# klindsay28/NK_ocn_tracer_jacobian_precond

Hardware: AMD Instinct MI355X
Metric: precond_solve_throughput_1deg_ocean_jacobian (higher is better)
Workload: dtype f64

## Files before the change

include/nkp.h:

```cpp
#ifndef NKP_H
#define NKP_H

#include <stdint.h>

#ifdef __cplusplus
extern "C" {
#endif

#define NKP_VERSION 1

typedef struct nkp_solver nkp_solver;

enum nkp_precond {
   NKP_PRECOND_NONE = 0,
   NKP_PRECOND_COLUMN_JACOBI = 1,
   NKP_PRECOND_MULTILEVEL = 3
};

enum nkp_krylov { NKP_KRYLOV_FGMRES = 0, NKP_KRYLOV_BICGSTAB = 1 };

enum {
   NKP_OK = 0,
   NKP_NOT_CONVERGED = 1,
   NKP_BREAKDOWN = 2,
   NKP_OK_BERR = 3,
   NKP_EINVAL = -1,
   NKP_ENOMEM = -2,
   NKP_EDEVICE = -3,
   NKP_ESINGULAR = -4,
   NKP_ECOMM = -5
};

typedef struct nkp_tuning {
   int struct_size;
   int ml_split;
   int ml_pocket;
   int ml_big_from;
   int ml_coarsest_rows;
   int ml_dense_max;
   double ml_theta;
   double ml_tau;
   int64_t ml_device_min;
   int ml_smooth_coarse;
   int ml_coarse_from;
   int ml_gamma_from, ml_gamma_to;
   int ml_f32;
   int ml_host_inverse;
   int ml_fused;
   int ml_fused_max_cols;
   int ml_wave_fused;
   int ml_coarsest_sweeps;
   int64_t ml_tail_rows;
   double ml_omega;
   int col_ldsres;
   int col_stream;
   int col_stream_min;
   int col_stream_gw;
   int col_wave_max;
   int col_w3;
   int col_group;
   int col_pipe_min;
   int col_ldsres_early;
   int col_ldsres_packed;
   int spmv_variant;
   int spmv_compress;
   int spmv_pipe_min;
   int spmv_run;
   int spmv_wgs;
   int rhs_batch;
   int precond_steps;
   int equil;
   int dist_overlap;
   int dist_ras;
   int force_dist;
   int setup_threads;
   int plan_times;
   int ml_drop_intertracer;
   int dist_one_reduce;
   int ml_huge_from;
   int col_ldsres_min;
   int col_sort_groups;
   int batch_spmv_rows;
   int dist_ras_rings;
   int ml_diag;
   int spmv_diag;
   int ml_lane_fused;
   int dist_smooth_exchange;
} nkp_tuning;

int nkp_default_tuning (nkp_tuning *t);

typedef struct nkp_options {
   int struct_size;
   int precond;
   int krylov;
   int restart;
   int max_iters;
   double rtol;
   double atol;
   int device;
   int verbose;
   int rank;
   int reorth;
   int ml_levels;
   int ml_smooth;
   int basis_f32;
   int precond_steps;
   int equil;
   int reserved[4];
   const int32_t *col_i;
   const int32_t *col_j;
   const int32_t *col_t;
   const nkp_tuning *tuning;
} nkp_options;

int nkp_default_options (nkp_options *opt);

int nkp_device_count (void);

int nkp_create (nkp_solver **out, const nkp_options *opt, int64_t n, int64_t nnz,
                const int32_t *rowptr, const int32_t *colind, const double *val,
                const int32_t *blk_start, int64_t nblk, int coupled_tracer_cnt);

int nkp_create64 (nkp_solver **out, const nkp_options *opt, int64_t n, const int64_t *rowptr ,
                  const int32_t *colind, const double *val, const int32_t *blk_start, int64_t nblk, int coupled_tracer_cnt);

int nkp_solve (nkp_solver *s, double *b_in_x_out, int nrhs, int64_t ldb,
               double *berr, int *iters, double *relres);

int nkp_solve_batch_device (nkp_solver *s, int nrhs, const void *d_B, void *d_X, int64_t ldb, double *berr, int *iters, double *relres);

int nkp_solve_device (nkp_solver *s, const void *d_b, void *d_x, int use_guess,
                      double *berr, int *iters, double *relres);

int nkp_spmv (nkp_solver *s, const double *x, double *y);
int nkp_spmv_device (nkp_solver *s, const void *d_x, void *d_y);

int nkp_precond_apply (nkp_solver *s, const double *r, double *z);

int nkp_multi_dot (nkp_solver *s, const double *V, int64_t ld, int k, const double *w, double *out);

int nkp_time_kernel (nkp_solver *s, int which, int arg, int reps, double *avg_ms);

int64_t nkp_get_int (nkp_solver *s, const char *key);

#define NKP_REFACTOR_REBUILD 1
int nkp_refactor (nkp_solver *s, const double *val, int flags);
int nkp_refactor_device (nkp_solver *s, const void *d_val, int flags);

int nkp_refactor_dist (nkp_solver *s, const double *val_loc, int flags);
int nkp_refactor_dist_device (nkp_solver *s, const void *d_val_loc, int flags);

int nkp_set_stream (nkp_solver *s, void *hip_stream);

void nkp_destroy (nkp_solver *s);

const char *nkp_last_error (void);


typedef struct nkp_comm_ops {
   void *ctx;
   int rank, nranks;
   int (*allreduce) (void *ctx, void *dev_buf, int count, int op, void *hip_stream);
   int (*alltoallv) (void *ctx, const void *dev_send, const int *send_counts, void *dev_recv, const int *recv_counts, void *hip_stream);
   int (*alltoallv_i32_host) (void *ctx, const int32_t *send, const int *send_counts, int32_t *recv, const int *recv_counts);
   int (*allgather_i64_host) (void *ctx, int64_t mine, int64_t *all );
} nkp_comm_ops;

int nkp_comm_unique_id (void *id128);
int nkp_comm_rccl_init (nkp_comm_ops *ops, const void *id128, int rank, int nranks);
void nkp_comm_rccl_free (nkp_comm_ops *ops);
int nkp_comm_file_init (nkp_comm_ops *ops, const char *dir, int rank, int nranks);
void nkp_comm_file_free (nkp_comm_ops *ops);

int nkp_create_dist (nkp_solver **out, const nkp_options *opt, int64_t n_global, int64_t fst_row,
                     int64_t m_loc, int64_t nnz_loc, const int32_t *rowptr_loc,
                     const int32_t *colind_glob, const double *val,
                     const int32_t *blk_start_loc, int64_t nblk_loc, int coupled_tracer_cnt,
                     const nkp_comm_ops *comm);

int nkp_cell_major_order (int64_t nblk, const int32_t *blk_start, int cnt, int32_t *perm, int32_t *blk_start_new,
                          int32_t *col_t, int32_t *col_src);
int nkp_permuted_rows (int64_t n, const int32_t *rowptr, const int32_t *colind, const double *val, const int32_t *perm,
                       const int32_t *inv, int64_t r0, int64_t r1, int32_t *rowptr_loc, int32_t *colind_loc, double *val_loc);

int nkp_clone (nkp_solver *src, nkp_solver **out);

int nkp_transpose (nkp_solver *s, nkp_solver **out);

int nkp_transpose_dist (nkp_solver *s, nkp_solver **out);

int nkp_value_gradient_device (nkp_solver *s, int nrhs, const void *d_lambda, const void *d_x, int64_t ld, double alpha, int accumulate, void *d_gval);
int nkp_value_gradient (nkp_solver *s, int nrhs, const double *lambda, const double *x, int64_t ld, double alpha, int accumulate, double *gval);

int nkp_values_product_device (nkp_solver *s, int nrhs, const void *d_val, const void *d_x, int64_t ldx, double alpha, int accumulate, void *d_y, int64_t ldy);
int nkp_values_product (nkp_solver *s, int nrhs, const double *val, const double *x, int64_t ldx, double alpha, int accumulate, double *y, int64_t ldy);

int nkp_solve_tangent_device (nkp_solver *s, int nrhs, const void *d_dval, const void *d_x, int64_t ldx, const void *d_db, void *d_dx, int64_t ld,
                              double *berr, int *iters, double *relres);

int nkp_set_device (int device);

int nkp_gather_root (nkp_solver *s, const double *x_loc, double *x_global);

typedef struct nkp_dist_plan nkp_dist_plan;
int nkp_dist_overlap_plan_host (nkp_dist_plan **out, const nkp_options *opt, int64_t n_global, int64_t fst_row, int64_t m_loc,
                                int64_t nnz_loc, const int32_t *rowptr_loc, const int32_t *colind_glob, const double *val,
                                const int32_t *blk_start_loc, int64_t nblk_loc, int coupled_tracer_cnt, const nkp_comm_ops *comm);
int64_t nkp_dist_plan_size (const nkp_dist_plan *p, const char *what);
int nkp_dist_plan_copy (const nkp_dist_plan *p, const char *what, void *dst);
void nkp_dist_plan_free (nkp_dist_plan *p);

int nkp_dist_plan_host (int64_t m_loc, int64_t nnz_loc, const int32_t *rowptr_loc, const int32_t *colind_glob,
                        int rank, int nranks, const int64_t *starts, int32_t *colind_ext, int32_t *halo_rows,
                        int64_t *n_halo, int32_t *need_counts);

int64_t nkp_ml_level_array (nkp_solver *s, int level, const char *what, void *dst, int64_t capacity_bytes);

int64_t nkp_matrix_array (nkp_solver *s, const char *what, void *dst, int64_t capacity_bytes);

int nkp_ml_plan_host (int64_t n, const int32_t *rowptr, const int32_t *colind, const double *val, const int32_t *blk_start,
                      int64_t nblk, const int32_t *col_i, const int32_t *col_j, int coupled_tracer_cnt, int max_levels,
                      int coarsest_rows, int64_t capacity, int *n_levels, int64_t *rows, int32_t *cmap, int32_t *col_of);

#ifdef __cplusplus
}
#endif
#endif
```

nk_ocn_tracer_jacobian_precond_amd/csrc/blas1.hip:

```cpp
#include "nkp_dev.h"

#include <stdint.h>

#define B1_THREADS 256

__device__ __forceinline__ double wave_sum (double v)
{
#pragma unroll
   for (int off = NKP_WAVE / 2; off > 0; off >>= 1) v += __shfl_down (v, off);
   return v;
}

__device__ __forceinline__ double block_sum (double v, double *sh )
{
   v = wave_sum (v);
   const int lane = threadIdx.x & (NKP_WAVE - 1), wv = threadIdx.x / NKP_WAVE;
   __syncthreads ();
   if (lane == 0) sh[wv] = v;
   __syncthreads ();
   double s = 0.0;
   if (threadIdx.x == 0) {
#pragma unroll
      for (int w = 0; w < B1_THREADS / NKP_WAVE; w++) s += sh[w];
   }
   return s;
}

static inline int red_grid (int64_t n)
{
   int64_t g = (n + 2 * B1_THREADS - 1) / (2 * B1_THREADS);
   if (g < 1) g = 1;
   if (g > NKP_RED_BLOCKS) g = NKP_RED_BLOCKS;
   return (int) g;
}

template <class VT, class VT2>
__device__ __forceinline__ void multi_dot_body (const VT *__restrict__ V, int64_t ld, int k, const double *__restrict__ w,
                                                int64_t n, double *__restrict__ partial, double *sh)
{
   const int chunk = blockIdx.y;
   const int j0 = chunk * NKP_DOT_CHUNK;
   const int kc = (k - j0) < NKP_DOT_CHUNK ? (k - j0) : NKP_DOT_CHUNK;
   const VT *Vc = V + (int64_t) j0 * ld;
   double acc[NKP_DOT_CHUNK];
#pragma unroll
   for (int c = 0; c < NKP_DOT_CHUNK; c++) acc[c] = 0.0;
   double accw = 0.0;
   const int64_t stride = (int64_t) gridDim.x * B1_THREADS * 2;
   for (int64_t i = ((int64_t) blockIdx.x * B1_THREADS + threadIdx.x) * 2; i < n; i += stride) {
      if (i + 1 < n) {
         const double2 w2 = *reinterpret_cast<const double2 *> (w + i);
         accw += w2.x * w2.x + w2.y * w2.y;
#pragma unroll
         for (int c = 0; c < NKP_DOT_CHUNK; c++)
            if (c < kc) {
               const VT2 v2 = *reinterpret_cast<const VT2 *> (Vc + (int64_t) c * ld + i);
               acc[c] += (double) v2.x * w2.x + (double) v2.y * w2.y;
            }
      } else {
         const double w1 = w[i];
         accw += w1 * w1;
#pragma unroll
         for (int c = 0; c < NKP_DOT_CHUNK; c++)
            if (c < kc) acc[c] += (double) Vc[(int64_t) c * ld + i] * w1;
      }
   }
   double *out = partial + ((int64_t) chunk * gridDim.x + blockIdx.x) * (NKP_DOT_CHUNK + 1);
#pragma unroll
   for (int c = 0; c < NKP_DOT_CHUNK; c++) {
      const double s = block_sum (acc[c], sh);
      if (threadIdx.x == 0) out[c] = s;
   }
   const double sw = block_sum (accw, sh);
   if (threadIdx.x == 0) out[NKP_DOT_CHUNK] = sw;
}

template <class VT, class VT2>
__global__ __launch_bounds__ (B1_THREADS)
void multi_dot_kernel (const VT *__restrict__ V, int64_t ld, int k, const double *__restrict__ w,
                       int64_t n, double *__restrict__ partial)
{
   __shared__ double sh[B1_THREADS / NKP_WAVE];
   multi_dot_body<VT, VT2> (V, ld, k, w, n, partial, sh);
}

__global__ __launch_bounds__ (B1_THREADS)
void multi_dot_group_kernel (GsGroup G, int64_t ld, int k, int64_t n)
{
   __shared__ double sh[B1_THREADS / NKP_WAVE];
   const int r = blockIdx.z;
   multi_dot_body<double, double2> (G.V[r], ld, k, G.w[r], n, G.partial[r], sh);
}

__device__ __forceinline__ void multi_dot_finish_body (const double *__restrict__ partial, int nblk, int k, double *__restrict__ out)
{
   const int j = blockIdx.x;
   const int chunk = (j < k) ? j / NKP_DOT_CHUNK : 0;
   const int c = (j < k) ? j % NKP_DOT_CHUNK : NKP_DOT_CHUNK;
   const double *p = partial + (int64_t) chunk * nblk * (NKP_DOT_CHUNK + 1) + c;
   double s = 0.0;
   for (int b = threadIdx.x; b < nblk; b += NKP_WAVE) s += p[(int64_t) b * (NKP_DOT_CHUNK + 1)];
   s = wave_sum (s);
   if (threadIdx.x == 0) out[j] = s;
}

__global__ __launch_bounds__ (NKP_WAVE)
void multi_dot_finish_kernel (const double *__restrict__ partial, int nblk, int k, double *__restrict__ out)
{
   multi_dot_finish_body (partial, nblk, k, out);
}

__global__ __launch_bounds__ (NKP_WAVE)
void multi_dot_finish_group_kernel (GsGroup G, int nblk, int k, double *__restrict__ msg)
{
   multi_dot_finish_body (G.partial[blockIdx.y], nblk, k, msg + (int64_t) blockIdx.y * (k + 1));
}

void launch_multi_dot (const void *V, int v_f32, int64_t ld, int k, const double *w, int64_t n, double *partial, double *out, hipStream_t st)
{
   const int g = red_grid (n);
   const int nchunk = k > 0 ? (k + NKP_DOT_CHUNK - 1) / NKP_DOT_CHUNK : 1;
   if (v_f32) hipLaunchKernelGGL ((multi_dot_kernel<float, float2>), dim3 (g, nchunk), dim3 (B1_THREADS), 0, st, (const float *) V, ld, k, w, n, partial);
   else hipLaunchKernelGGL ((multi_dot_kernel<double, double2>), dim3 (g, nchunk), dim3 (B1_THREADS), 0, st, (const double *) V, ld, k, w, n, partial);
   hipLaunchKernelGGL (multi_dot_finish_kernel, dim3 (k + 1), dim3 (NKP_WAVE), 0, st, partial, g, k, out);
}

void launch_multi_dot_group (int R, const GsGroup &G, int64_t ld, int k, int64_t n, double *msg, hipStream_t st)
{
   if (R <= 0) return;
   const int g = red_grid (n);
   const int nchunk = k > 0 ? (k + NKP_DOT_CHUNK - 1) / NKP_DOT_CHUNK : 1;
   hipLaunchKernelGGL (multi_dot_group_kernel, dim3 (g, nchunk, R), dim3 (B1_THREADS), 0, st, G, ld, k, n);
   hipLaunchKernelGGL (multi_dot_finish_group_kernel, dim3 (k + 1, R), dim3 (NKP_WAVE), 0, st, G, g, k, msg);
}

#define B1_MAX_K NKP_MAX_K
template <class VT, class VT2>
__device__ __forceinline__ void update_w_body (const VT *__restrict__ V, int64_t ld, int k, const double *__restrict__ h,
                                               double *__restrict__ w, int64_t n, double *__restrict__ partial, double sign, double *hs, double *sh)
{
   for (int j = threadIdx.x; j < k; j += B1_THREADS) hs[j] = sign * h[j];
   __syncthreads ();
   double nrm = 0.0;
   const int64_t stride = (int64_t) gridDim.x * B1_THREADS * 2;
   for (int64_t i = ((int64_t) blockIdx.x * B1_THREADS + threadIdx.x) * 2; i < n; i += stride) {
      if (i + 1 < n) {
         double2 a = *reinterpret_cast<const double2 *> (w + i);
         int j = 0;
         for (; j + 4 <= k; j += 4) {
            const VT2 v0 = *reinterpret_cast<const VT2 *> (V + (int64_t) (j + 0) * ld + i);
            const VT2 v1 = *reinterpret_cast<const VT2 *> (V + (int64_t) (j + 1) * ld + i);
            const VT2 v2 = *reinterpret_cast<const VT2 *> (V + (int64_t) (j + 2) * ld + i);
            const VT2 v3 = *reinterpret_cast<const VT2 *> (V + (int64_t) (j + 3) * ld + i);
            a.x += hs[j] * v0.x; a.y += hs[j] * v0.y;
            a.x += hs[j + 1] * v1.x; a.y += hs[j + 1] * v1.y;
            a.x += hs[j + 2] * v2.x; a.y += hs[j + 2] * v2.y;
            a.x += hs[j + 3] * v3.x; a.y += hs[j + 3] * v3.y;
         }
         for (; j < k; j++) {
            const VT2 v0 = *reinterpret_cast<const VT2 *> (V + (int64_t) j * ld + i);
            a.x += hs[j] * v0.x; a.y += hs[j] * v0.y;
         }
         *reinterpret_cast<double2 *> (w + i) = a;
         nrm += a.x * a.x + a.y * a.y;
      } else {
         double a = w[i];
         for (int j = 0; j < k; j++) a += hs[j] * V[(int64_t) j * ld + i];
         w[i] = a;
         nrm += a * a;
      }
   }
   if (partial) {
      const double s = block_sum (nrm, sh);
      if (threadIdx.x == 0) partial[blockIdx.x] = s;
   }
}

template <class VT, class VT2>
__global__ __launch_bounds__ (B1_THREADS)
void update_w_kernel (const VT *__restrict__ V, int64_t ld, int k, const double *__restrict__ h,
                      double *__restrict__ w, int64_t n, double *__restrict__ partial, double sign)
{
   __shared__ double hs[B1_MAX_K];
   __shared__ double sh[B1_THREADS / NKP_WAVE];
   update_w_body<VT, VT2> (V, ld, k, h, w, n, partial, sign, hs, sh);
}

__global__ __launch_bounds__ (B1_THREADS)
void update_w_group_kernel (GsGroup G, int64_t ld, int k, const double *__restrict__ msg, int64_t n)
{
   __shared__ double hs[B1_MAX_K];
   __shared__ double sh[B1_THREADS / NKP_WAVE];
   const int r = blockIdx.y;
   update_w_body<double, double2> (G.V[r], ld, k, msg + (int64_t) r * (k + 1), G.w[r], n, G.partial[r], -1.0, hs, sh);
}

__device__ __forceinline__ void sum_partials_body (const double *__restrict__ partial, int nblk, double *__restrict__ out)
{
   double s = 0.0;
   for (int b = threadIdx.x; b < nblk; b += NKP_WAVE) s += partial[b];
   s = wave_sum (s);
   if (threadIdx.x == 0) out[0] = s;
}

__global__ __launch_bounds__ (NKP_WAVE)
void sum_partials_kernel (const double *__restrict__ partial, int nblk, double *__restrict__ out)
{
   sum_partials_body (partial, nblk, out);
}

__global__ __launch_bounds__ (NKP_WAVE)
void sum_partials_group_kernel (GsGroup G, int nblk, double *__restrict__ out)
{
   sum_partials_body (G.partial[blockIdx.x], nblk, out + blockIdx.x);
}

void launch_update_w (const void *V, int v_f32, int64_t ld, int k, const double *h, double *w, int64_t n, double *partial, double *out_nrm2, hipStream_t st)
{
   const int g = red_grid (n);
   if (v_f32) hipLaunchKernelGGL ((update_w_kernel<float, float2>), dim3 (g), dim3 (B1_THREADS), 0, st, (const float *) V, ld, k, h, w, n, partial, -1.0);
   else hipLaunchKernelGGL ((update_w_kernel<double, double2>), dim3 (g), dim3 (B1_THREADS), 0, st, (const double *) V, ld, k, h, w, n, partial, -1.0);
   hipLaunchKernelGGL (sum_partials_kernel, dim3 (1), dim3 (NKP_WAVE), 0, st, partial, g, out_nrm2);
}

void launch_update_w_group (int R, const GsGroup &G, int64_t ld, int k, const double *msg, int64_t n, double *nrm2, hipStream_t st)
{
   if (R <= 0) return;
   const int g = red_grid (n);
   hipLaunchKernelGGL (update_w_group_kernel, dim3 (g, R), dim3 (B1_THREADS), 0, st, G, ld, k, msg, n);
   hipLaunchKernelGGL (sum_partials_group_kernel, dim3 (R), dim3 (NKP_WAVE), 0, st, G, g, nrm2);
}

void launch_axpy_multi (const double *Z, int64_t ld, int k, const double *c, double *x, int64_t n, hipStream_t st)
{
   const int g = red_grid (n);
   hipLaunchKernelGGL ((update_w_kernel<double, double2>), dim3 (g), dim3 (B1_THREADS), 0, st, Z, ld, k, c, x, n, (double *) nullptr, 1.0);
}

__device__ __forceinline__ void scale_to_body (const double *__restrict__ x, const double *__restrict__ alpha, double *__restrict__ y, float *__restrict__ yf, int64_t n)
{
   const double a = alpha[0];
   const int64_t stride = (int64_t) gridDim.x * B1_THREADS * 2;
   for (int64_t i = ((int64_t) blockIdx.x * B1_THREADS + threadIdx.x) * 2; i < n; i += stride) {
      if (i + 1 < n) {
         double2 v = *reinterpret_cast<const double2 *> (x + i);
         v.x *= a; v.y *= a;
         *reinterpret_cast<double2 *> (y + i) = v;
         if (yf) *reinterpret_cast<float2 *> (yf + i) = make_float2 ((float) v.x, (float) v.y);
      } else {
         y[i] = a * x[i];
         if (yf) yf[i] = (float) (a * x[i]);
      }
   }
}

__global__ __launch_bounds__ (B1_THREADS)
void scale_to_kernel (const double *__restrict__ x, const double *__restrict__ alpha, double *__restrict__ y, float *__restrict__ yf, int64_t n)
{
   scale_to_body (x, alpha, y, yf, n);
}

__global__ __launch_bounds__ (B1_THREADS)
void scale_to_group_kernel (GsGroup G, const double *__restrict__ inv, int64_t n)
{
   const int r = blockIdx.y;
   scale_to_body (G.w[r], inv + r, G.vnext[r], nullptr, n);
}

void launch_scale_to (const double *x, const double *alpha_dev, double *y, float *yf, int64_t n, hipStream_t st)
{
   hipLaunchKernelGGL (scale_to_kernel, dim3 (red_grid (n)), dim3 (B1_THREADS), 0, st, x, alpha_dev, y, yf, n);
}

void launch_scale_to_group (int R, const GsGroup &G, const double *inv, int64_t n, hipStream_t st)
{
   if (R > 0) hipLaunchKernelGGL (scale_to_group_kernel, dim3 (red_grid (n), R), dim3 (B1_THREADS), 0, st, G, inv, n);
}

__global__ __launch_bounds__ (B1_THREADS)
void axpby_kernel (double a, const double *__restrict__ x, double b, double *__restrict__ y, int64_t n)
{
   const int64_t stride = (int64_t) gridDim.x * B1_THREADS;
   for (int64_t i = (int64_t) blockIdx.x * B1_THREADS + threadIdx.x; i < n; i += stride)
      y[i] = (b == 0.0 ? 0.0 : b * y[i]) + (x ? a * x[i] : a);
}

void launch_axpby (double a, const double *x, double b, double *y, int64_t n, hipStream_t st)
{
   hipLaunchKernelGGL (axpby_kernel, dim3 (red_grid (n) * 2), dim3 (B1_THREADS), 0, st, a, x, b, y, n);
}

__global__ __launch_bounds__ (B1_THREADS)
void vmul_kernel (const double *x, const double *__restrict__ w, double *y, int64_t n)
{
   const int64_t stride = (int64_t) gridDim.x * B1_THREADS;
   for (int64_t i = (int64_t) blockIdx.x * B1_THREADS + threadIdx.x; i < n; i += stride) y[i] = x[i] * w[i];
}

void launch_vmul (const double *x, const double *w, double *y, int64_t n, hipStream_t st)
{
   hipLaunchKernelGGL (vmul_kernel, dim3 (red_grid (n) * 2), dim3 (B1_THREADS), 0, st, x, w, y, n);
}

void launch_copy (const double *x, double *y, int64_t n, hipStream_t st)
{
   (void) hipMemcpyAsync (y, x, (size_t) n * sizeof (double), hipMemcpyDeviceToDevice, st);
}

__global__ __launch_bounds__ (B1_THREADS)
void zero_kernel (double *__restrict__ y, int64_t n)
{
   const int64_t stride = (int64_t) gridDim.x * B1_THREADS * 2;
   for (int64_t i = ((int64_t) blockIdx.x * B1_THREADS + threadIdx.x) * 2; i < n; i += stride) {
      if (i + 1 < n) *reinterpret_cast<double2 *> (y + i) = make_double2 (0.0, 0.0);
      else y[i] = 0.0;
   }
}

void launch_fill (double *y, double v, int64_t n, hipStream_t st)
{
   if (n <= 0) return;
   if (v == 0.0) {
      if ((reinterpret_cast<uintptr_t> (y) & 15) == 0) hipLaunchKernelGGL (zero_kernel, dim3 (red_grid (n) * 2), dim3 (B1_THREADS), 0, st, y, n);
      else (void) hipMemsetAsync (y, 0, (size_t) n * sizeof (double), st);
   } else
      launch_axpby (v, nullptr, 0.0, y, n, st);
}

__global__ __launch_bounds__ (B1_THREADS)
void dot_kernel (const double *__restrict__ x, const double *__restrict__ y, int64_t n, double *__restrict__ partial)
{
   __shared__ double sh[B1_THREADS / NKP_WAVE];
   double acc = 0.0;
   const int64_t stride = (int64_t) gridDim.x * B1_THREADS * 2;
   for (int64_t i = ((int64_t) blockIdx.x * B1_THREADS + threadIdx.x) * 2; i < n; i += stride) {
      if (i + 1 < n) {
         const double2 a = *reinterpret_cast<const double2 *> (x + i);
         const double2 b = *reinterpret_cast<const double2 *> (y + i);
         acc += a.x * b.x + a.y * b.y;
      } else
         acc += x[i] * y[i];
   }
   const double s = block_sum (acc, sh);
   if (threadIdx.x == 0) partial[blockIdx.x] = s;
}

void launch_dot (const double *x, const double *y, int64_t n, double *partial, double *out, hipStream_t st)
{
   const int g = red_grid (n);
   hipLaunchKernelGGL (dot_kernel, dim3 (g), dim3 (B1_THREADS), 0, st, x, y, n, partial);
   hipLaunchKernelGGL (sum_partials_kernel, dim3 (1), dim3 (NKP_WAVE), 0, st, partial, g, out);
}

__device__ __forceinline__ double max_or_nan (double q, double m)
{
   return (q > m || q != q) ? q : m;
}

__global__ __launch_bounds__ (B1_THREADS)
void berr_kernel (const double *__restrict__ r, const double *__restrict__ den, int64_t n, double *__restrict__ partial)
{
   __shared__ double sh[B1_THREADS / NKP_WAVE];
   double m = 0.0;
   const int64_t stride = (int64_t) gridDim.x * B1_THREADS;
   for (int64_t i = (int64_t) blockIdx.x * B1_THREADS + threadIdx.x; i < n; i += stride) {
      const double a = fabs (r[i]), d = den[i];
      const double q = (d > 0.0 || d != d) ? a / d : (a != a ? a : a > 0.0 ? 1.0e300 : 0.0);
      m = max_or_nan (q, m);
   }
   for (int off = NKP_WAVE / 2; off > 0; off >>= 1) m = max_or_nan (__shfl_down (m, off), m);
   const int lane = threadIdx.x & (NKP_WAVE - 1), wv = threadIdx.x / NKP_WAVE;
   if (lane == 0) sh[wv] = m;
   __syncthreads ();
   if (threadIdx.x == 0) {
      for (int w = 1; w < B1_THREADS / NKP_WAVE; w++) m = max_or_nan (sh[w], m);
      partial[blockIdx.x] = m;
   }
}

__global__ __launch_bounds__ (NKP_WAVE)
void max_partials_kernel (const double *__restrict__ partial, int nblk, double *__restrict__ out)
{
   double m = 0.0;
   for (int b = threadIdx.x; b < nblk; b += NKP_WAVE) m = max_or_nan (partial[b], m);
   for (int off = NKP_WAVE / 2; off > 0; off >>= 1) m = max_or_nan (__shfl_down (m, off), m);
   if (threadIdx.x == 0) out[0] = m;
}

void launch_berr (const double *r, const double *den, int64_t n, double *partial, double *out, hipStream_t st)
{
   const int g = red_grid (n);
   hipLaunchKernelGGL (berr_kernel, dim3 (g), dim3 (B1_THREADS), 0, st, r, den, n, partial);
   hipLaunchKernelGGL (max_partials_kernel, dim3 (1), dim3 (NKP_WAVE), 0, st, partial, g, out);
}

__global__ __launch_bounds__ (B1_THREADS)
void count_entries_kernel (const double *__restrict__ x, int64_t n, double *__restrict__ partial)
{
   __shared__ double sh[B1_THREADS / NKP_WAVE];
   double bad = 0.0, set = 0.0;
   const int64_t stride = (int64_t) gridDim.x * B1_THREADS;
   for (int64_t i = (int64_t) blockIdx.x * B1_THREADS + threadIdx.x; i < n; i += stride) {
      const double v = x[i];
      bad += (v - v == 0.0) ? 0.0 : 1.0;
      set += (v == 0.0) ? 0.0 : 1.0;
   }
   const double sb = block_sum (bad, sh);
   if (threadIdx.x == 0) partial[blockIdx.x] = sb;
   const double ss = block_sum (set, sh);
   if (threadIdx.x == 0) partial[NKP_RED_BLOCKS + blockIdx.x] = ss;
}

void launch_count_entries (const double *x, int64_t n, double *partial, double *out, hipStream_t st)
{
   const int g = red_grid (n);
   hipLaunchKernelGGL (count_entries_kernel, dim3 (g), dim3 (B1_THREADS), 0, st, x, n, partial);
   hipLaunchKernelGGL (sum_partials_kernel, dim3 (1), dim3 (NKP_WAVE), 0, st, partial, g, out);
   hipLaunchKernelGGL (sum_partials_kernel, dim3 (1), dim3 (NKP_WAVE), 0, st, partial + NKP_RED_BLOCKS, g, out + 1);
}

__device__ __forceinline__ void finish_column_body (double *__restrict__ h, const double *__restrict__ h2, int k,
                                                    const double *__restrict__ nrm2, double *__restrict__ inv)
{
   if (h2)
      for (int j = threadIdx.x; j < k; j += NKP_WAVE) h[j] += h2[j];
   if (threadIdx.x == 0) {
      const double t = sqrt (nrm2[0]);
      h[k] = t;
      inv[0] = (t > 0.0) ? 1.0 / t : 0.0;
   }
}

__global__ __launch_bounds__ (NKP_WAVE)
void finish_column_kernel (double *__restrict__ h, const double *__restrict__ h2, int k,
                           const double *__restrict__ nrm2, double *__restrict__ inv)
{
   finish_column_body (h, h2, k, nrm2, inv);
}

__device__ __forceinline__ void finish_column_pythagoras_body (double *__restrict__ h, int k, double *__restrict__ inv)
{
   double s = 0.0;
   for (int j = threadIdx.x; j < k; j += NKP_WAVE) s += h[j] * h[j];
   for (int off = NKP_WAVE / 2; off > 0; off >>= 1) s += __shfl_down (s, off);
   if (threadIdx.x == 0) {
      const double ww = h[k];
      double t2 = ww - s;
      const bool weak = !(t2 >= 1e-8 * ww);
      if (!(t2 > 0.0)) t2 = 0.0;
      const double t = sqrt (t2);
      h[k] = weak ? -t : t;
      inv[0] = (t > 0.0) ? 1.0 / t : 0.0;
   }
}

__global__ __launch_bounds__ (NKP_WAVE)
void finish_column_pythagoras_kernel (double *__restrict__ h, int k, double *__restrict__ inv)
{
   finish_column_pythagoras_body (h, k, inv);
}

__global__ __launch_bounds__ (NKP_WAVE)
void finish_column_group_kernel (double *__restrict__ msg, const double *__restrict__ msg2, int k, const double *__restrict__ nrm2, double *__restrict__ inv)
{
   const int64_t r = blockIdx.x;
   if (nrm2) finish_column_body (msg + r * (k + 1), msg2 ? msg2 + r * (k + 1) : nullptr, k, nrm2 + r, inv + r);
   else finish_column_pythagoras_body (msg + r * (k + 1), k, inv + r);
}

void launch_finish_column_group (int R, double *msg, const double *msg2, int k, const double *nrm2, double *inv, hipStream_t st)
{
   if (R > 0) hipLaunchKernelGGL (finish_column_group_kernel, dim3 (R), dim3 (NKP_WAVE), 0, st, msg, msg2, k, nrm2, inv);
}

void launch_finish_column_pythagoras (double *h, int k, double *inv, hipStream_t st)
{
   hipLaunchKernelGGL (finish_column_pythagoras_kernel, dim3 (1), dim3 (NKP_WAVE), 0, st, h, k, inv);
}

void launch_finish_column (double *h, const double *h2, int k, const double *nrm2, double *inv, hipStream_t st)
{
   hipLaunchKernelGGL (finish_column_kernel, dim3 (1), dim3 (NKP_WAVE), 0, st, h, h2, k, nrm2, inv);
}

__global__ __launch_bounds__ (B1_THREADS)
void restrict_sum_kernel (const int *__restrict__ rptr, const int *__restrict__ ridx, const double *__restrict__ fine,
                          double *__restrict__ coarse, int64_t nc)
{
   const int64_t stride = (int64_t) gridDim.x * B1_THREADS;
   for (int64_t I = (int64_t) blockIdx.x * B1_THREADS + threadIdx.x; I < nc; I += stride) {
      double acc = 0.0;
      for (int q = rptr[I]; q < rptr[I + 1]; q++) acc += fine[ridx[q]];
      coarse[I] = acc;
   }
}

void launch_restrict_sum (const int *rptr, const int *ridx, const double *fine, double *coarse, int64_t nc, hipStream_t st)
{
   if (nc <= 0) return;
   hipLaunchKernelGGL (restrict_sum_kernel, dim3 (red_grid (nc) * 2), dim3 (B1_THREADS), 0, st, rptr, ridx, fine, coarse, nc);
}

__global__ __launch_bounds__ (B1_THREADS)
void prolong_add_kernel (const int *__restrict__ cmap, const double *__restrict__ coarse, double *__restrict__ fine, int64_t nf, double omega)
{
   const int64_t stride = (int64_t) gridDim.x * B1_THREADS;
   for (int64_t i = (int64_t) blockIdx.x * B1_THREADS + threadIdx.x; i < nf; i += stride) fine[i] += omega * coarse[cmap[i]];
}

void launch_prolong_add (const int *cmap, const double *coarse, double *fine, int64_t nf, double omega, hipStream_t st)
{
   if (nf <= 0) return;
   hipLaunchKernelGGL (prolong_add_kernel, dim3 (red_grid (nf) * 2), dim3 (B1_THREADS), 0, st, cmap, coarse, fine, nf, omega);
}

__global__ __launch_bounds__ (B1_THREADS)
void gather_kernel (const int *__restrict__ perm, const double *__restrict__ in, double *__restrict__ out, int64_t n, int scatter)
{
   const int64_t stride = (int64_t) gridDim.x * B1_THREADS;
   for (int64_t i = (int64_t) blockIdx.x * B1_THREADS + threadIdx.x; i < n; i += stride) {
      if (scatter) out[perm[i]] = in[i];
      else out[i] = in[perm[i]];
   }
}

void launch_gather (const int *perm, const double *in, double *out, int64_t n, hipStream_t st)
{
   if (n <= 0) return;
   hipLaunchKernelGGL (gather_kernel, dim3 (red_grid (n) * 2), dim3 (B1_THREADS), 0, st, perm, in, out, n, 0);
}

void launch_scatter (const int *perm, const double *in, double *out, int64_t n, hipStream_t st)
{
   if (n <= 0) return;
   hipLaunchKernelGGL (gather_kernel, dim3 (red_grid (n) * 2), dim3 (B1_THREADS), 0, st, perm, in, out, n, 1);
}

__global__ __launch_bounds__ (B1_THREADS)
void dense_matvec_kernel (const double *__restrict__ M, const double *__restrict__ x, double *__restrict__ y, int n)
{
   const int row = (int) ((blockIdx.x * B1_THREADS + threadIdx.x) / NKP_WAVE);
   const int lane = threadIdx.x & (NKP_WAVE - 1);
   if (row >= n) return;
   const double *m = M + (int64_t) row * n;
   double acc = 0.0;
   for (int c = lane; c < n; c += NKP_WAVE) acc += m[c] * x[c];
   acc = wave_sum (acc);
   if (lane == 0) y[row] = acc;
}

void launch_dense_matvec (const double *Minv, const double *x, double *y, int n, hipStream_t st)
{
   if (n <= 0) return;
   const int waves_per_block = B1_THREADS / NKP_WAVE;
   hipLaunchKernelGGL (dense_matvec_kernel, dim3 ((n + waves_per_block - 1) / waves_per_block), dim3 (B1_THREADS), 0, st, Minv, x, y, n);
}
```

nk_ocn_tracer_jacobian_precond_amd/csrc/inspect.hip:

```cpp
#include "solver_impl.h"

#include <string.h>

#include <vector>

extern "C" int64_t nkp_ml_level_array (nkp_solver *s, int level, const char *what, void *dst, int64_t capacity_bytes)
{
   if (!s || !what || s->opt.precond != NKP_PRECOND_MULTILEVEL || level < 0 || level >= (int) s->ml.lev.size ()) return fail (NKP_EINVAL, "nkp_ml_level_array: bad argument");
   const MlLevel &V = s->ml.lev[(size_t) level];
   const bool last = level == (int) s->ml.lev.size () - 1;
   const void *src = nullptr;
   int64_t count = 0;
   size_t elem = 4;
   bool host = false;
   int col_kernel[11];
   if (!strcmp (what, "rowptr")) { src = V.L.rowptr; count = V.n + 1; }
   else if (!strcmp (what, "colind")) { src = V.L.colind; count = V.L.nnz; }
   else if (!strcmp (what, "valf")) { src = V.L.valf; count = V.L.valf ? V.L.nnz : 0; }
   else if (!strcmp (what, "val")) { src = V.L.val; count = V.L.val ? V.L.nnz : 0; elem = 8; }
   else if (!strcmp (what, "dg_ptr")) { src = V.L.dg_ptr; count = src ? V.L.dg_ncol + 1 : 0; }
   else if (!strcmp (what, "dg_key")) { src = V.L.dg_key; count = src ? (int64_t) V.L.dg_nkey : 0; }
   else if (!strcmp (what, "dg_voff")) { src = V.L.dg_voff; count = src ? V.L.dg_ncol : 0; elem = 8; }
   else if (!strcmp (what, "dg_val")) { src = V.L.dg_val; count = src ? V.L.dg_nval : 0; }
   else if (!strcmp (what, "dg_gptr")) { src = V.L.dg_gptr; count = src ? V.L.dg_ncol + 1 : 0; }
   else if (!strcmp (what, "dg_grp")) { src = V.L.dg_grp; count = src ? 2 * (int64_t) V.L.dg_ngrp : 0; }
   else if (!strcmp (what, "cmap")) { src = V.cmap; count = V.cmap ? V.n : 0; }
   else if (!strcmp (what, "rptr")) { src = V.rptr; count = V.rptr ? V.nc + 1 : 0; }
   else if (!strcmp (what, "ridx")) { src = V.ridx; count = V.ridx ? V.n : 0; }
   else if (!strcmp (what, "blk_start")) { src = V.B.blk_start; count = V.B.blk_start ? V.B.nblk + 1 : 0; }
   else if (!strcmp (what, "fac")) { src = V.B.fac; count = V.B.fac ? (int64_t) (2 * V.B.P + 1) * V.n : 0; elem = 8; }
   else if (!strcmp (what, "perm0")) { src = level == 0 ? s->ml.perm0 : nullptr; count = src ? V.n : 0; }
   else if (!strcmp (what, "coarse_inv")) { src = last ? s->ml.coarse_inv : nullptr; count = src ? V.n * V.n : 0; elem = 8; }
   else if (!strcmp (what, "color_blk")) { src = V.B.blk_start ? V.color_blk : nullptr; count = src ? 3 : 0; host = true; }
   else if (!strcmp (what, "col_kernel")) {
      const ColBlocksDev &B = V.B;
      const int v[11] = { V.wave_columns ? 1 : 0, V.wave_fused ? 1 : 0, B.stream ? 1 : 0, B.ldsres, B.gw, B.P, B.dropped, B.max_len, B.gs_ok, B.ngrp, B.lds_doubles };
      memcpy (col_kernel, v, sizeof v);
      src = B.blk_start ? col_kernel : nullptr; count = src ? 11 : 0; host = true;
   }
   else if (!strcmp (what, "wave_diag")) { src = &V.wave_diag; count = 1; host = true; }
   else if (!strcmp (what, "lane_diag")) { src = &V.lane_diag; count = 1; host = true; }
   else if (!strcmp (what, "grp_tile")) { src = V.B.grp_tile; count = src ? (int64_t) V.B.ngrp * V.B.gw : 0; }
   else return fail (NKP_EINVAL, "nkp_ml_level_array: unknown array '%s'", what);
   if (!dst) return count;
   if (count * (int64_t) elem > capacity_bytes) return fail (NKP_EINVAL, "nkp_ml_level_array: buffer too small");
   if (host) {
      if (count) memcpy (dst, src, (size_t) count * elem);
      return count;
   }
   HIPCHK (hipSetDevice (s->device));
   HIPCHK (hipStreamSynchronize (s->stream));
   if (count) HIPCHK (hipMemcpy (dst, src, (size_t) count * elem, hipMemcpyDeviceToHost));
   return count;
}

extern "C" int64_t nkp_matrix_array (nkp_solver *s, const char *what, void *dst, int64_t capacity_bytes)
{
   if (!s || !what) return fail (NKP_EINVAL, "nkp_matrix_array: bad argument");
   const CsrDev &A = s->A;
   const bool have = A.dg_vald != nullptr;
   const void *src = nullptr;
   int64_t count = 0;
   size_t elem = 4;
   if (!strcmp (what, "dg_ptr")) { src = A.dg_ptr; count = have ? A.dg_ncol + 1 : 0; }
   else if (!strcmp (what, "dg_key")) { src = A.dg_key; count = have ? (int64_t) A.dg_nkey : 0; }
   else if (!strcmp (what, "dg_voff")) { src = A.dg_voff; count = have ? A.dg_ncol : 0; elem = 8; }
   else if (!strcmp (what, "dg_val")) { src = A.dg_vald; count = have ? A.dg_nval : 0; elem = 8; }
   else if (!strcmp (what, "dg_gptr")) { src = A.dg_gptr; count = have ? A.dg_ncol + 1 : 0; }
   else if (!strcmp (what, "dg_grp")) { src = A.dg_grp; count = have ? 2 * (int64_t) A.dg_ngrp : 0; }
   else if (!strcmp (what, "rowptr")) { src = A.rowptr; count = src ? A.n + 1 : 0; }
   else if (!strcmp (what, "colind")) { src = A.colind; count = src ? A.nnz : 0; }
   else if (!strcmp (what, "val")) { src = A.val; count = src ? A.nnz : 0; elem = 8; }
   else if (!strcmp (what, "fac")) { src = s->opt.precond == NKP_PRECOND_COLUMN_JACOBI ? s->B.fac : nullptr; count = src ? (int64_t) (2 * s->B.P + 1) * s->B.n : 0; elem = 8; }
   else return fail (NKP_EINVAL, "nkp_matrix_array: unknown array '%s'", what);
   if (!dst) return count;
   if (count * (int64_t) elem > capacity_bytes) return fail (NKP_EINVAL, "nkp_matrix_array: buffer too small");
   HIPCHK (hipSetDevice (s->device));
   HIPCHK (hipStreamSynchronize (s->stream));
   if (count) HIPCHK (hipMemcpy (dst, src, (size_t) count * elem, hipMemcpyDeviceToHost));
   return count;
}

extern "C" int nkp_spmv_device (nkp_solver *s, const void *d_x, void *d_y)
{
   if (!s || !d_x || !d_y) return fail (NKP_EINVAL, "nkp_spmv_device: NULL argument");
   HIPCHK (hipSetDevice (s->device));
   spmv_op (s, (const double *) d_x, (double *) d_y, nullptr, 0);
   HIPCHK (hipStreamSynchronize (s->stream));
   HIPCHK (hipGetLastError ());
   return NKP_OK;
}

extern "C" int nkp_spmv (nkp_solver *s, const double *x, double *y)
{
   if (!s || !x || !y) return fail (NKP_EINVAL, "nkp_spmv: NULL argument");
   HIPCHK (hipSetDevice (s->device));
   const size_t bytes = (size_t) s->n * sizeof (double);
   HIPCHK (hipMemcpyAsync (s->t1, x, bytes, hipMemcpyHostToDevice, s->stream));
   spmv_op (s, s->t1, s->t2, nullptr, 0);
   HIPCHK (hipMemcpyAsync (y, s->t2, bytes, hipMemcpyDeviceToHost, s->stream));
   HIPCHK (hipStreamSynchronize (s->stream));
   HIPCHK (hipGetLastError ());
   return NKP_OK;
}

extern "C" int nkp_precond_apply (nkp_solver *s, const double *r, double *z)
{
   if (!s || !r || !z) return fail (NKP_EINVAL, "nkp_precond_apply: NULL argument");
   if (s->shared->broken) return refactor_broken (s);
   HIPCHK (hipSetDevice (s->device));
   const size_t bytes = (size_t) s->n * sizeof (double);
   HIPCHK (hipMemcpyAsync (s->t1, r, bytes, hipMemcpyHostToDevice, s->stream));
   apply_precond_once (s, s->t1, s->t2);
   HIPCHK (hipMemcpyAsync (z, s->t2, bytes, hipMemcpyDeviceToHost, s->stream));
   HIPCHK (hipStreamSynchronize (s->stream));
   HIPCHK (hipGetLastError ());
   return NKP_OK;
}

extern "C" int nkp_multi_dot (nkp_solver *s, const double *V, int64_t ld, int k, const double *w, double *out)
{
   if (!s || !V || !w || !out || k < 0 || k > s->m + 1 || ld < s->n) return fail (NKP_EINVAL, "nkp_multi_dot: bad argument (k must be <= restart+1)");
   HIPCHK (hipSetDevice (s->device));
   std::vector<float> vf;
   for (int j = 0; j < k; j++) {
      if (s->vf32) {
         vf.assign (V + (int64_t) j * ld, V + (int64_t) j * ld + s->n);
         HIPCHK (hipMemcpyAsync ((float *) s->V + (int64_t) j * s->ld, vf.data (), (size_t) s->n * sizeof (float), hipMemcpyHostToDevice, s->stream));
         HIPCHK (hipStreamSynchronize (s->stream));
      } else
         HIPCHK (hipMemcpyAsync (s->V + (int64_t) j * s->ld, V + (int64_t) j * ld, (size_t) s->n * sizeof (double), hipMemcpyHostToDevice, s->stream));
   }
   HIPCHK (hipMemcpyAsync (s->w, w, (size_t) s->n * sizeof (double), hipMemcpyHostToDevice, s->stream));
   launch_multi_dot (s->V, s->vf32, s->ld, k, s->w, s->n, s->partial, s->h_dev (), s->stream);
   allreduce_dev (s, s->h_dev (), k + 1, 0);
   HIPCHK (hipMemcpyAsync (out, s->h_dev (), (size_t) (k + 1) * sizeof (double), hipMemcpyDeviceToHost, s->stream));
   HIPCHK (hipStreamSynchronize (s->stream));
   HIPCHK (hipGetLastError ());
   return NKP_OK;
}

extern "C" int nkp_time_kernel (nkp_solver *s, int which, int arg, int reps, double *avg_ms)
{
   if (!s || !avg_ms || reps < 1) return fail (NKP_EINVAL, "nkp_time_kernel: bad argument");
   if (which == 8 && !s->A.dg_vald) return fail (NKP_EINVAL, "nkp_time_kernel: the matrix has no per-column diagonals (tuning spmv_diag)");
   HIPCHK (hipSetDevice (s->device));
   if (which == 5) {
      const int prc = valgrad_time_prepare (s, arg);
      if (prc) return prc;
   }
   if (which == 6 || which == 7) {
      const int prc = valprod_time_prepare (s, arg, which);
      if (prc) return prc;
   }
   hipEvent_t e0, e1;
   HIPCHK (hipEventCreate (&e0));
   HIPCHK (hipEventCreate (&e1));
   launch_fill (s->t1, 1.0, s->n, s->stream);
   if (which == 2) {
      if (arg < 0 || arg >= s->m) return fail (NKP_EINVAL, "nkp_time_kernel: restart position out of range");
      for (int j = 0; j <= arg + 1; j++) {
         launch_fill (s->t2, 1.0 / (1.0 + j), s->n, s->stream);
         s->hpin[0] = 1.0;
         HIPCHK (hipMemcpyAsync (s->misc_dev () + 1, s->hpin, sizeof (double), hipMemcpyHostToDevice, s->stream));
         if (s->vf32) launch_scale_to (s->t2, s->misc_dev () + 1, s->vcur, (float *) s->V + (int64_t) j * s->ld, s->n, s->stream);
         else launch_scale_to (s->t2, s->misc_dev () + 1, s->V + (int64_t) j * s->ld, nullptr, s->n, s->stream);
         HIPCHK (hipStreamSynchronize (s->stream));
      }
   }
   for (int pass = 0; pass < 2; pass++) {
      const int cnt = pass == 0 ? (reps < 3 ? reps : 3) : reps;
      HIPCHK (hipEventRecord (e0, s->stream));
      for (int i = 0; i < cnt; i++) {
         if (which == 0 && s->A.dg_vald) launch_csr_spmv (s->A, s->t1, s->t2, nullptr, 0, s->stream);
         else if (which == 0) spmv_op (s, s->t1, s->t2, nullptr, 0);
         else if (which == 8) launch_diag_spmv (s->A, s->t1, s->t2, nullptr, 0, s->stream);
         else if (which == 1) apply_precond_once (s, s->t1, s->t2);
         else if (which == 2) arnoldi_step_device (s, arg);
         else if (which == 5) valgrad_time_launch (s, arg);
         else if (which == 6) valprod_time_launch (s, arg);
         else if (which == 7) valprod_time_composition (s, arg);
         else if (s->opt.precond == NKP_PRECOND_MULTILEVEL) ml_time_piece (s->ml, which - 3, s->stream);
      }
      HIPCHK (hipEventRecord (e1, s->stream));
      HIPCHK (hipEventSynchronize (e1));
      float ms = 0.f;
      HIPCHK (hipEventElapsedTime (&ms, e0, e1));
      *avg_ms = (double) ms / cnt;
   }
   (void) hipEventDestroy (e0);
   (void) hipEventDestroy (e1);
   HIPCHK (hipGetLastError ());
   return NKP_OK;
}
```

nk_ocn_tracer_jacobian_precond_amd/csrc/krylov.hip:

```cpp
#include "solver_impl.h"

#include <math.h>

void apply_precond_once (nkp_solver *s, const double *rin, double *zout)
{
   if (s->opt.precond == NKP_PRECOND_NONE) launch_copy (rin, zout, s->n, s->stream);
   else if (s->opt.precond == NKP_PRECOND_MULTILEVEL && s->dist.ras) {
      if (s->dist.ras_sep) {
         if (s->dist.ras_nsend) launch_gather (s->dist.ras_send_idx, rin, s->dist.ras_sendbuf, s->dist.ras_nsend, s->stream);
         alltoallv_dev (s, s->dist.ras_sendbuf, s->dist.ras_send_counts.data (), s->dist.rext + s->n, s->dist.ras_recv_counts.data (), s->stream);
         launch_copy (rin, s->dist.rext, s->n, s->stream);
      } else {
         if (s->dist.nsend) launch_gather (s->dist.send_idx, rin, s->dist.sendbuf, s->dist.nsend, s->stream);
         alltoallv_dev (s, s->dist.sendbuf, s->dist.send_counts.data (), s->dist.xe + s->n, s->dist.recv_counts.data (), s->stream);
         launch_copy (rin, s->dist.rext, s->n, s->stream);
         if (s->dist.n_sel) launch_gather (s->dist.sel_idx, s->dist.xe + s->n, s->dist.rext + s->n, s->dist.n_sel, s->stream);
      }
      ml_apply (s->ml, s->dist.rext, s->dist.zext, s->stream, smooth_hook_of (s));
      launch_copy (s->dist.zext, zout, s->n, s->stream);
   } else if (s->opt.precond == NKP_PRECOND_MULTILEVEL) ml_apply (s->ml, rin, zout, s->stream);
   else launch_colblock_apply_lanes (s->B, 0, s->B.ngrp, rin, zout, 0, s->stream);
}

void apply_precond (nkp_solver *s, const double *rin, double *zout)
{
   apply_precond_once (s, rin, zout);
   for (int k = 1; k < s->steps_now && s->p1 && s->p2; k++) {
      spmv_op (s, zout, s->p1, rin, 1);
      apply_precond_once (s, s->p1, s->p2);
      launch_axpby (1.0, s->p2, 1.0, zout, s->n, s->stream);
   }
}

void spmv_op (nkp_solver *s, const double *x, double *y, const double *b, int mode)
{
   const double *xin = x;
   if (s->dist.on) {
      launch_copy (x, s->dist.xe, s->n, s->stream);
      if (s->dist.nsend) launch_gather (s->dist.send_idx, x, s->dist.sendbuf, s->dist.nsend, s->stream);
      xin = s->dist.xe;
      if (s->dist.overlap) {
         (void) hipEventRecord (s->dist.ev_packed, s->stream);
         (void) hipStreamWaitEvent (s->dist.comm_stream, s->dist.ev_packed, 0);
         alltoallv_dev (s, s->dist.sendbuf, s->dist.send_counts.data (), s->dist.xe + s->n, s->dist.recv_counts.data (), s->dist.comm_stream);
         (void) hipEventRecord (s->dist.ev_halo, s->dist.comm_stream);
         launch_csr_spmv_range (s->A, s->dist.seg_rb[1], s->dist.seg_rb[2], xin, y, b, mode, s->stream);
         (void) hipStreamWaitEvent (s->stream, s->dist.ev_halo, 0);
         launch_csr_spmv_range (s->A, s->dist.seg_rb[0], s->dist.seg_rb[1], xin, y, b, mode, s->stream);
         launch_csr_spmv_range (s->A, s->dist.seg_rb[2], s->dist.seg_rb[3], xin, y, b, mode, s->stream);
         return;
      }
      alltoallv_dev (s, s->dist.sendbuf, s->dist.send_counts.data (), s->dist.xe + s->n, s->dist.recv_counts.data (), s->stream);
   }
   if (mode == 2) launch_csr_abs_spmv (s->A, xin, b, y, s->stream);
   else if (s->A.dg_vald) launch_diag_spmv (s->A, xin, y, b, mode, s->stream);
   else launch_csr_spmv (s->A, xin, y, b, mode, s->stream);
}

static int dot_host (nkp_solver *s, const double *x, const double *y, double *out)
{
   launch_dot (x, y, s->n, s->partial, s->misc_dev () + 2, s->stream);
   allreduce_dev (s, s->misc_dev () + 2, 1, 0);
   HIPCHK (hipMemcpyAsync (s->hpin, s->misc_dev () + 2, sizeof (double), hipMemcpyDeviceToHost, s->stream));
   HIPCHK (hipStreamSynchronize (s->stream));
   if (s->comm_failed) return fail (NKP_ECOMM, "nkp_solve: a collective of the distributed solve failed");
   *out = s->hpin[0];
   return NKP_OK;
}

void arnoldi_apply (nkp_solver *s, int j)
{
   const int64_t ld = s->ld;
   double *zj = s->Z + (int64_t) j * ld;
   const double *vj = s->vf32 ? s->vcur : s->V + (int64_t) j * ld;
   if (s->equil) {
      launch_vmul (vj, s->rinv, s->eqtmp, s->n, s->stream);
      apply_precond (s, s->eqtmp, zj);
      spmv_op (s, zj, s->w, nullptr, 0);
      launch_vmul (s->w, s->rscale, s->w, s->n, s->stream);
   } else {
      apply_precond (s, vj, zj);
      spmv_op (s, zj, s->w, nullptr, 0);
   }
}

void arnoldi_orthogonalise (nkp_solver *s, int j)
{
   const int64_t ld = s->ld;
   launch_multi_dot (s->V, s->vf32, ld, j + 1, s->w, s->n, s->partial, s->h_dev (), s->stream);
   allreduce_dev (s, s->h_dev (), j + 2, 0);
   launch_update_w (s->V, s->vf32, ld, j + 1, s->h_dev (), s->w, s->n, s->partial, s->misc_dev (), s->stream);
   if (s->opt.reorth) {
      launch_multi_dot (s->V, s->vf32, ld, j + 1, s->w, s->n, s->partial, s->h2_dev (), s->stream);
      allreduce_dev (s, s->h2_dev (), j + 2, 0);
      launch_update_w (s->V, s->vf32, ld, j + 1, s->h2_dev (), s->w, s->n, s->partial, s->misc_dev (), s->stream);
      allreduce_dev (s, s->misc_dev (), 1, 0);
      launch_finish_column (s->h_dev (), s->h2_dev (), j + 1, s->misc_dev (), s->misc_dev () + 1, s->stream);
   } else if (s->dist.on && s->tune.dist_one_reduce) {
      launch_finish_column_pythagoras (s->h_dev (), j + 1, s->misc_dev () + 1, s->stream);
   } else {
      allreduce_dev (s, s->misc_dev (), 1, 0);
      launch_finish_column (s->h_dev (), nullptr, j + 1, s->misc_dev (), s->misc_dev () + 1, s->stream);
   }
   if (s->vf32) launch_scale_to (s->w, s->misc_dev () + 1, s->vcur, (float *) s->V + (int64_t) (j + 1) * ld, s->n, s->stream);
   else launch_scale_to (s->w, s->misc_dev () + 1, s->V + (int64_t) (j + 1) * ld, nullptr, s->n, s->stream);
}

void arnoldi_step_device (nkp_solver *s, int j)
{
   arnoldi_apply (s, j);
   arnoldi_orthogonalise (s, j);
}


int rhs_refused (int verdict, const char *what)
{
   if (verdict == RHS_NONFINITE) return fail (NKP_BREAKDOWN, "%s holds a non-finite entry (NaN or Inf): not solved, x is NaN", what);
   return fail (NKP_BREAKDOWN, "%s is outside the range of the solve (||b||^2 finite in f64 and max (rtol ||b||, atol) >= 2^-480 = 3.2e-145): "
                               "not solved, x is NaN; scale the system", what);
}

static int classify_rhs (nkp_solver *s, double bnorm2, double target, int *verdict)
{
   double nonfinite = 0.0, nonzero = 0.0;
   if (rhs_needs_counts (bnorm2, target)) {
      launch_count_entries (s->b, s->n, s->partial, s->misc_dev () + 4, s->stream);
      allreduce_dev (s, s->misc_dev () + 4, 2, 0);
      HIPCHK (hipMemcpyAsync (s->hpin, s->misc_dev () + 4, 2 * sizeof (double), hipMemcpyDeviceToHost, s->stream));
      HIPCHK (hipStreamSynchronize (s->stream));
      if (s->comm_failed) return fail (NKP_ECOMM, "nkp_solve: a collective of the distributed solve failed");
      nonfinite = s->hpin[0];
      nonzero = s->hpin[1];
   }
   s->rhs_class = *verdict = rhs_verdict (bnorm2, target, nonfinite, nonzero);
   if (*verdict == RHS_ZERO) launch_fill (s->x, 0.0, s->n, s->stream);
   else if (*verdict != RHS_ORDINARY) launch_fill (s->x, NAN, s->n, s->stream);
   return NKP_OK;
}

int fg_begin (nkp_solver *s, FgmresState &F)
{
   fg_init (F, s->m);
   double bnorm2 = 0.0;
   int rc = dot_host (s, s->b, s->b, &bnorm2);
   if (rc) return rc;
   F.bnorm = sqrt (bnorm2);
   F.target = fmax (s->opt.rtol * F.bnorm, s->opt.atol);
   s->stagnated = false;
   s->steps_now = s->precond_steps;
   int verdict = RHS_ORDINARY;
   if ((rc = classify_rhs (s, bnorm2, F.target, &verdict))) return rc;
   if (verdict != RHS_ORDINARY) {
      F.finished = true;
      F.status = verdict == RHS_ZERO ? NKP_OK : NKP_BREAKDOWN;
      F.relres = verdict == RHS_ZERO ? 0.0 : NAN;
   }
   return NKP_OK;
}

int fg_restart (nkp_solver *s, FgmresState &F)
{
   hipStream_t st = s->stream;
   const int64_t n = s->n;
   int rc;
   spmv_op (s, s->x, s->r, s->b, 1);
   double r2 = 0.0;
   if ((rc = dot_host (s, s->r, s->r, &r2))) return rc;
   const double beta = sqrt (r2);
   const int todo = fg_restart_verdict (F, beta, s->opt.max_iters, s->steps_now);
   msg (s, 2, "fgmres: its = %d, true relres = %.3e\n", F.its, F.relres);
   if (s->comm_failed) return fail (NKP_ECOMM, "nkp_solve: a collective of the distributed solve failed");
   if (todo & FG_LOWER_STEPS) {
      msg (s, 1, "fgmres: no progress over a restart cycle with %d preconditioner cycles per iteration; continuing with one\n", s->steps_now);
      s->steps_now = 1;
   }
   if (todo & FG_STAGNATED) s->stagnated = true;
   if (todo & FG_STOP) return NKP_OK;
   if (s->equil) {
      launch_vmul (s->r, s->rscale, s->r, n, st);
      double q2 = 0.0;
      if ((rc = dot_host (s, s->r, s->r, &q2))) return rc;
      F.beta_it = sqrt (q2);
      if (!(F.beta_it > 0.0)) { F.status = NKP_BREAKDOWN; F.finished = true; return NKP_OK; }
      F.target_it = F.target * (F.beta_it / beta);
   }
   s->hpin[0] = 1.0 / F.beta_it;
   HIPCHK (hipMemcpyAsync (s->misc_dev () + 1, s->hpin, sizeof (double), hipMemcpyHostToDevice, st));
   if (s->vf32) launch_scale_to (s->r, s->misc_dev () + 1, s->vcur, (float *) s->V, n, st);
   else launch_scale_to (s->r, s->misc_dev () + 1, s->V, nullptr, n, st);
   HIPCHK (hipStreamSynchronize (st));
   fg_start_cycle (F);
   return NKP_OK;
}

bool fg_post_step (nkp_solver *s, FgmresState &F)
{
   const bool ends = fg_column_step (F, s->hpin, s->opt.max_iters);
   if (!F.breakdown_in_cycle) msg (s, 3, "fgmres: its = %d, est relres = %.3e\n", F.its, F.est / F.bnorm);
   return ends;
}

int fg_end_cycle (nkp_solver *s, FgmresState &F)
{
   const int k = F.j;
   hipStream_t st = s->stream;
   fg_back_substitute (F);
   for (int i = 0; i < k; i++) s->hpin[i] = F.y[i];
   HIPCHK (hipMemcpyAsync (s->y_dev (), s->hpin, (size_t) k * sizeof (double), hipMemcpyHostToDevice, st));
   launch_axpy_multi (s->Z, s->ld, k, s->y_dev (), s->x, s->n, st);
   HIPCHK (hipStreamSynchronize (st));
   if (F.breakdown_in_cycle) {
      int rc;
      double r2 = 0.0;
      spmv_op (s, s->x, s->r, s->b, 1);
      if ((rc = dot_host (s, s->r, s->r, &r2))) return rc;
      F.relres = is_finite (r2) ? sqrt (r2) / F.bnorm : NAN;
      F.status = sqrt (r2) <= F.target ? NKP_OK : NKP_BREAKDOWN;
      F.finished = true;
   }
   return NKP_OK;
}

static int fgmres (nkp_solver *s, int *iters_out, double *relres_out)
{
   FgmresState F;
   int rc = fg_begin (s, F);
   if (rc) return rc;
   while (!F.finished) {
      if ((rc = fg_restart (s, F))) return rc;
      if (F.finished) break;
      for (;;) {
         arnoldi_step_device (s, F.j);
         HIPCHK (hipMemcpyAsync (s->hpin, s->h_dev (), (size_t) (F.j + 2) * sizeof (double), hipMemcpyDeviceToHost, s->stream));
         HIPCHK (hipStreamSynchronize (s->stream));
         if (s->comm_failed) return fail (NKP_ECOMM, "nkp_solve: a collective of the distributed solve failed (Arnoldi step %d)", F.its + 1);
         if (fg_post_step (s, F)) break;
      }
      if ((rc = fg_end_cycle (s, F))) return rc;
   }
   HIPCHK (hipGetLastError ());
   *iters_out = F.its;
   *relres_out = F.relres;
   return F.status;
}

static int bicgstab (nkp_solver *s, int *iters_out, double *relres_out)
{
   const int64_t n = s->n, ld = s->ld;
   hipStream_t st = s->stream;
   if (s->m < 2) return fail (NKP_EINVAL, "bicgstab needs restart >= 2 (it borrows the Krylov basis storage)");
   double *r = s->r, *r0 = s->V, *p = s->V + ld, *v = s->V + 2 * ld;
   double *ph = s->Z, *sh = s->Z + ld, *t = s->t2, *sv = s->t1;
   int rc;
   double bnorm2, rho = 1.0, alpha = 1.0, omega = 1.0, tmp;
   if ((rc = dot_host (s, s->b, s->b, &bnorm2))) return rc;
   const double bnorm = sqrt (bnorm2);
   const double target = fmax (s->opt.rtol * bnorm, s->opt.atol);
   int verdict = RHS_ORDINARY;
   if ((rc = classify_rhs (s, bnorm2, target, &verdict))) return rc;
   if (verdict != RHS_ORDINARY) {
      *iters_out = 0;
      *relres_out = verdict == RHS_ZERO ? 0.0 : NAN;
      return verdict == RHS_ZERO ? NKP_OK : NKP_BREAKDOWN;
   }
   spmv_op (s, s->x, r, s->b, 1);
   launch_copy (r, r0, n, st);
   launch_fill (p, 0.0, n, st);
   launch_fill (v, 0.0, n, st);
   int its = 0, status = NKP_NOT_CONVERGED;
   double rn2;
   if ((rc = dot_host (s, r, r, &rn2))) return rc;
   double relres = sqrt (rn2) / bnorm;
   while (its < s->opt.max_iters) {
      if (!is_finite (rn2)) { status = NKP_BREAKDOWN; break; }
      if (sqrt (rn2) <= target) { status = NKP_OK; break; }
      double rho_new;
      if ((rc = dot_host (s, r0, r, &rho_new))) return rc;
      if (rho_new == 0.0 || !(rho_new == rho_new)) { status = NKP_BREAKDOWN; break; }
      const double beta = (rho_new / rho) * (alpha / omega);
      launch_axpby (-omega, v, 1.0, p, n, st);
      launch_axpby (1.0, r, beta, p, n, st);
      apply_precond (s, p, ph);
      spmv_op (s, ph, v, nullptr, 0);
      if ((rc = dot_host (s, r0, v, &tmp))) return rc;
      if (tmp == 0.0 || !(tmp == tmp)) { status = NKP_BREAKDOWN; break; }
      alpha = rho_new / tmp;
      launch_copy (r, sv, n, st);
      launch_axpby (-alpha, v, 1.0, sv, n, st);
      apply_precond (s, sv, sh);
      spmv_op (s, sh, t, nullptr, 0);
      double ts, tt;
      if ((rc = dot_host (s, t, sv, &ts))) return rc;
      if ((rc = dot_host (s, t, t, &tt))) return rc;
      if (tt == 0.0 || !(tt == tt)) { status = NKP_BREAKDOWN; break; }
      omega = ts / tt;
      launch_axpby (alpha, ph, 1.0, s->x, n, st);
      launch_axpby (omega, sh, 1.0, s->x, n, st);
      launch_copy (sv, r, n, st);
      launch_axpby (-omega, t, 1.0, r, n, st);
      rho = rho_new;
      its++;
      if ((rc = dot_host (s, r, r, &rn2))) return rc;
      relres = sqrt (rn2) / bnorm;
      msg (s, 3, "bicgstab: its = %d, recurrence relres = %.3e\n", its, relres);
      if (omega == 0.0) { status = NKP_BREAKDOWN; break; }
   }
   spmv_op (s, s->x, r, s->b, 1);
   if ((rc = dot_host (s, r, r, &rn2))) return rc;
   relres = sqrt (rn2) / bnorm;
   if (!is_finite (rn2)) { relres = NAN; status = NKP_BREAKDOWN; }
   else if (sqrt (rn2) <= target * 1.0001) status = NKP_OK;
   else if (status == NKP_OK) status = NKP_NOT_CONVERGED;
   HIPCHK (hipGetLastError ());
   *iters_out = its;
   *relres_out = relres;
   return status;
}

int backward_error (nkp_solver *s, double *berr)
{
   spmv_op (s, s->x, s->r, s->b, 1);
   spmv_op (s, s->x, s->t1, s->b, 2);
   launch_berr (s->r, s->t1, s->n, s->partial, s->misc_dev () + 3, s->stream);
   allreduce_dev (s, s->misc_dev () + 3, 1, 1);
   HIPCHK (hipMemcpyAsync (s->hpin, s->misc_dev () + 3, sizeof (double), hipMemcpyDeviceToHost, s->stream));
   HIPCHK (hipStreamSynchronize (s->stream));
   *berr = s->hpin[0];
   return NKP_OK;
}

static int solve_resident (nkp_solver *s, double *berr, int *iters, double *relres)
{
   if (s->shared->broken) return refactor_broken (s);
   int it = 0;
   double rr = 0.0;
   s->stagnated = false;
   int status = (s->opt.krylov == NKP_KRYLOV_BICGSTAB) ? bicgstab (s, &it, &rr) : fgmres (s, &it, &rr);
   if (status < 0) return status;
   double be = 0.0;
   if (berr || s->stagnated) {
      int rc = backward_error (s, &be);
      if (rc) return rc;
      if (berr) *berr = be;
   }
   if (s->comm_failed) return fail (NKP_ECOMM, "nkp_solve: a collective of the distributed solve failed");
   if (status == NKP_NOT_CONVERGED && s->stagnated && be <= fmax (NKP_BERR_ROUNDING_LEVEL, 1.0e-2 * s->opt.rtol)) {
      msg (s, 1, "nkp_solve: residual stagnated at %.3e (rtol %.1e) with backward error %.3e: NKP_OK_BERR\n", rr, s->opt.rtol, be);
      status = NKP_OK_BERR;
   }
   if (iters) *iters = it;
   if (relres) *relres = rr;
   msg (s, 1, "nkp_solve: %s after %d iterations, ||b-Ax||/||b|| = %.3e\n", status == NKP_OK ? "converged" : status == NKP_OK_BERR ? "at the attainable accuracy (backward error accepted)" : status == NKP_BREAKDOWN ? "breakdown" : "NOT converged", it, rr);
   if (s->rhs_class == RHS_NONFINITE || s->rhs_class == RHS_OUT_OF_RANGE) rhs_refused (s->rhs_class, "nkp_solve: the right-hand side");
   else if (status == NKP_OK_BERR) fail (status, "nkp_solve: ||b-Ax||/||b|| = %.3e stopped above rtol %.1e at the attainable accuracy after %d iterations; componentwise backward error %.3e", rr, s->opt.rtol, it, be);
   else if (status != NKP_OK) fail (status, "nkp_solve: %s after %d iterations (relres %.3e, rtol %.1e)", status == NKP_BREAKDOWN ? "breakdown" : s->stagnated ? "stagnated at the attainable accuracy, not converged" : "not converged", it, rr, s->opt.rtol);
   return status;
}

extern "C" int nkp_solve_device (nkp_solver *s, const void *d_b, void *d_x, int use_guess, double *berr, int *iters, double *relres)
{
   if (!s || !d_b || !d_x) return fail (NKP_EINVAL, "nkp_solve_device: NULL argument");
   HIPCHK (hipSetDevice (s->device));
   const size_t bytes = (size_t) s->n * sizeof (double);
   if (use_guess) HIPCHK (hipMemcpyAsync (s->x, d_x, bytes, hipMemcpyDeviceToDevice, s->stream));
   else HIPCHK (hipMemsetAsync (s->x, 0, bytes, s->stream));
   HIPCHK (hipMemcpyAsync (s->b, d_b, bytes, hipMemcpyDeviceToDevice, s->stream));
   int status = solve_resident (s, berr, iters, relres);
   if (status < 0) return status;
   HIPCHK (hipMemcpyAsync (d_x, s->x, bytes, hipMemcpyDeviceToDevice, s->stream));
   HIPCHK (hipStreamSynchronize (s->stream));
   return status;
}

extern "C" int nkp_solve (nkp_solver *s, double *b_in_x_out, int nrhs, int64_t ldb, double *berr, int *iters, double *relres)
{
   if (!s || (nrhs > 0 && !b_in_x_out)) return fail (NKP_EINVAL, "nkp_solve: NULL argument");
   if (nrhs < 0 || (nrhs > 0 && ldb < s->n)) return fail (NKP_EINVAL, "nkp_solve: bad nrhs/ldb");
   HIPCHK (hipSetDevice (s->device));
   const size_t bytes = (size_t) s->n * sizeof (double);
   int worst = NKP_OK;
   if (nrhs >= 2 && s->tune.rhs_batch && !batch_unsupported (s)) {
      double *dB = nullptr;
      const int64_t ldd = s->ld;
      int status = NKP_OK;
      if (hipMalloc ((void **) &dB, (size_t) ldd * (size_t) nrhs * sizeof (double)) != hipSuccess) {
         dB = nullptr;
         (void) hipGetLastError ();
         status = fail (NKP_ENOMEM, "nkp_solve: device memory for %d right-hand sides", nrhs);
      }
      for (int c = 0; c < nrhs && status == NKP_OK; c++)
         if (hipMemcpy (dB + (size_t) c * (size_t) ldd, b_in_x_out + (size_t) c * (size_t) ldb, bytes, hipMemcpyHostToDevice) != hipSuccess) status = fail (NKP_EDEVICE, "nkp_solve: upload of right-hand side %d failed", c);
      if (s->dist.on) status = dist_agree (s, status, "nkp_solve", "staging the right-hand sides on the device");
      if (status != NKP_OK) { if (dB) (void) hipFree (dB); return status; }
      if (status == NKP_OK) status = nkp_solve_batch_device (s, nrhs, dB, dB, ldd, berr, iters, relres);
      if (status >= 0)
         for (int c = 0; c < nrhs; c++)
            if (hipMemcpy (b_in_x_out + (size_t) c * (size_t) ldb, dB + (size_t) c * (size_t) ldd, bytes, hipMemcpyDeviceToHost) != hipSuccess) status = fail (NKP_EDEVICE, "nkp_solve: download of solution %d failed", c);
      (void) hipFree (dB);
      return status;
   }
   if (nrhs >= 2 && s->tune.rhs_batch) note_fallback (s, "nkp_solve", batch_unsupported (s), nrhs);
   for (int c = 0; c < nrhs; c++) {
      double *col = b_in_x_out + (size_t) c * (size_t) ldb;
      HIPCHK (hipMemcpyAsync (s->b, col, bytes, hipMemcpyHostToDevice, s->stream));
      HIPCHK (hipMemsetAsync (s->x, 0, bytes, s->stream));
      int status = solve_resident (s, berr ? berr + c : nullptr, iters ? iters + c : nullptr, relres ? relres + c : nullptr);
      if (status < 0) return status;
      HIPCHK (hipMemcpyAsync (col, s->x, bytes, hipMemcpyDeviceToHost, s->stream));
      HIPCHK (hipStreamSynchronize (s->stream));
      if (sev_of (status) > sev_of (worst)) worst = status;
   }
   return worst;
}
```

nk_ocn_tracer_jacobian_precond_amd/csrc/mlcycle.hip:

```cpp
#include "nkp_dev.h"
#include "multilevel.h"

static void column_solves (const MlHierarchy &H, MlLevel &V, int c, const double *rhs, double *x, int accumulate, hipStream_t st)
{
   if (V.wave_columns) {
      if (H.f32) launch_colblock_apply_range_r32 (V.B, V.color_blk[c], V.color_blk[c + 1], rhs, x, accumulate, st);
      else launch_colblock_apply_range (V.B, V.color_blk[c], V.color_blk[c + 1], rhs, x, accumulate, st);
   } else
      launch_colblock_apply_lanes (V.B, V.color_grp[c], V.color_grp[c + 1], rhs, x, accumulate, st);
}

static inline void after_half_sweep (MlHierarchy &H, const MlLevel &V, int c, double *x, int K, hipStream_t st)
{
   if (!H.hook || &V != &H.lev[0] || H.hook_left <= 0) return;
   if (--H.hook_left > 0) H.hook->refresh (H.hook->ctx, c, x, K, st);
}

static void gs_half (MlHierarchy &H, MlLevel &V, int c, bool fused, hipStream_t st)
{
   if (fused) {
      const int out = (V.cur[0] != V.cur[1]) ? V.cur[1 - c] : 1 - V.cur[c];
      const int rows0 = (int) V.rows0;
      if (V.wave_diag) launch_gs_wave_diag (V.L, V.B, V.color_tile[c], V.color_tile[c + 1], V.xbuf (V.cur[0]), V.xbuf (V.cur[1]), rows0, V.b, V.xbuf (out), H.f32, st);
      else if (V.lane_diag) launch_gs_lanes_diag (V.L, V.B, V.color_grp[c], V.color_grp[c + 1], V.xbuf (V.cur[0]), V.xbuf (V.cur[1]), rows0, V.b, V.xbuf (out), st);
      else if (V.wave_fused) launch_gs_wave (V.L, V.B, V.color_blk[c], V.color_blk[c + 1], V.xbuf (V.cur[0]), V.xbuf (V.cur[1]), rows0, V.b, V.xbuf (out), H.f32, st);
      else (void) launch_gs_fused (V.L, V.B, V.color_grp[c], V.color_grp[c + 1], V.xbuf (V.cur[0]), V.xbuf (V.cur[1]), rows0, V.b, V.xbuf (out), st);
      V.cur[c] = out;
      after_half_sweep (H, V, c, V.xbuf (out), 1, st);
      return;
   }
   if (V.L.dg_val) launch_diag_residual (V.L, V.color_tile[c], V.color_tile[c + 1], V.x, V.b, V.r, st);
   else launch_csr_residual_range (V.L, V.color_rb[c], V.color_rb[c + 1], V.x, V.b, V.r, st);
   column_solves (H, V, c, V.r, V.x, 1, st);
   after_half_sweep (H, V, c, V.x, 1, st);
}

static void gs_sweep (MlHierarchy &H, MlLevel &V, bool reverse, bool fused, hipStream_t st)
{
   for (int step = 0; step < 2; step++) gs_half (H, V, reverse ? 1 - step : step, fused, st);
}

static void ml_cycle (MlHierarchy &H, int l, hipStream_t st)
{
   MlLevel &V = H.lev[l];
   V.cur[0] = V.cur[1] = 0;
   if (l == 0) H.hook_left = 0;
   if (l == H.tail_from && H.coarse_inv && H.gamma_to <= H.gamma_from && ml_tail_launch (H, l, st) == 0) return;
   if (l == (int) H.lev.size () - 1) {
      if (H.coarse_inv) {
         if (H.coarse_invf) launch_dense_matvec_f32 (H.coarse_invf, H.coarse_ldf, V.b, V.x, (int) V.n, st);
         else launch_dense_matvec (H.coarse_inv, V.b, V.x, (int) V.n, st);
         return;
      }
      const int sweeps = H.tune->ml_coarsest_sweeps > 0 ? H.tune->ml_coarsest_sweeps : 30;
      launch_fill (V.x, 0.0, V.n, st);
      column_solves (H, V, 0, V.b, V.x, 0, st);
      gs_half (H, V, 1, false, st);
      for (int s = 1; s < sweeps; s++) gs_sweep (H, V, s & 1, false, st);
      return;
   }
   const bool fused = ml_level_fused (H, V);
   const int nu = (l >= H.coarse_from) ? H.nu_coarse : H.nu;
   if (l == 0 && H.hook) H.hook_left = 4 * nu;
   launch_fill (V.x, 0.0, V.n, st);
   if (fused) {
      if (V.wave_fused) column_solves (H, V, 0, V.b, V.x2, 0, st);
      else launch_colblock_apply_lanes (V.B, V.color_grp[0], V.color_grp[1], V.b, V.x2, 0, st);
      V.cur[0] = 1;
      after_half_sweep (H, V, 0, V.x2, 1, st);
      gs_half (H, V, 1, true, st);
   } else {
      column_solves (H, V, 0, V.b, V.x, 0, st);
      after_half_sweep (H, V, 0, V.x, 1, st);
      gs_half (H, V, 1, false, st);
   }
   for (int s = 1; s < nu; s++) gs_sweep (H, V, false, fused, st);
   MlLevel &C = H.lev[l + 1];
   const int gamma = (l >= H.gamma_from && l < H.gamma_to) ? 2 : 1;
   for (int g = 0; g < gamma; g++) {
      if (V.L.dg_val) launch_diag_residual (V.L, V.color_tile[0], V.color_tile[2], V.xnow (), V.b, V.r, st);
      else launch_csr_spmv (V.L, V.xnow (), V.r, V.b, 1, st);
      launch_restrict_sum (V.rptr, V.ridx, V.r, C.b, V.nc, st);
      ml_cycle (H, l + 1, st);
      launch_prolong_add (V.cmap, C.xnow (), V.xnow (), V.n, H.omega, st);
   }
   for (int s = 0; s < nu; s++) gs_sweep (H, V, true, fused, st);
}

void ml_apply (MlHierarchy &H, const double *r, double *z, hipStream_t st, const MlSmoothHook *hook)
{
   MlLevel &V = H.lev[0];
   launch_gather (H.perm0, r, V.b, V.n, st);
   H.hook = hook;
   ml_cycle (H, 0, st);
   H.hook = nullptr;
   launch_scatter (H.perm0, V.xnow (), z, V.n, st);
}

int ml_batch_prepare (MlHierarchy &H, int K)
{
   if (K != 2 && K != 4 && K != 8) return -1;
   if (H.batch_K >= K) return 0;
   auto drop = [&H] () {
      for (MlLevel &V : H.lev)
         for (double **p : { &V.bx, &V.bx2, &V.bb, &V.br })
            if (*p) {
               (void) hipFree (*p);
               *p = nullptr;
               H.device_bytes -= (size_t) (V.n ? V.n : 1) * (size_t) H.batch_K * sizeof (double);
            }
      H.batch_K = 0;
   };
   drop ();
   for (MlLevel &V : H.lev) {
      for (double **p : { &V.bx, &V.bx2, &V.bb, &V.br }) {
         const size_t bytes = (size_t) (V.n ? V.n : 1) * (size_t) K * sizeof (double);
         void *q = nullptr;
         if (hipMalloc (&q, bytes) != hipSuccess || hipMemset (q, 0, bytes) != hipSuccess) {
            if (q) (void) hipFree (q);
            H.batch_K = K;
            drop ();
            (void) hipGetLastError ();
            return -2;
         }
         *p = (double *) q;
         H.device_bytes += bytes;
      }
   }
   H.batch_K = K;
   return 0;
}

static void column_solves_batch (const MlHierarchy &H, MlLevel &V, int K, int c, const double *rhs, double *x, int accumulate, hipStream_t st)
{
   if (launch_colblock_apply_lanes_batch (K, V.B, V.color_grp[c], V.color_grp[c + 1], rhs, x, accumulate, st) != 0)
      launch_colblock_apply_wave_batch (K, V.B, V.color_blk[c], V.color_blk[c + 1], rhs, x, accumulate, H.f32, st);
}

static void gs_half_batch (MlHierarchy &H, MlLevel &V, int K, int c, hipStream_t st)
{
   if (V.wave_fused) {
      const int out = (V.bcur[0] != V.bcur[1]) ? V.bcur[1 - c] : 1 - V.bcur[c];
      launch_gs_wave_batch (K, V.L, V.B, V.color_blk[c], V.color_blk[c + 1], V.bxbuf (V.bcur[0]), V.bxbuf (V.bcur[1]), (int) V.rows0, V.bb, V.bxbuf (out), H.f32, st);
      V.bcur[c] = out;
      after_half_sweep (H, V, c, V.bxbuf (out), K, st);
      return;
   }
   launch_csr_spmv_batch (K, V.L, V.color_rb[c], V.color_rb[c + 1], V.bx, V.br, V.bb, 1, st);
   column_solves_batch (H, V, K, c, V.br, V.bx, 1, st);
   after_half_sweep (H, V, c, V.bx, K, st);
}

static void ml_cycle_batch (MlHierarchy &H, int K, int l, hipStream_t st)
{
   MlLevel &V = H.lev[l];
   const int64_t nk = V.n * K;
   V.bcur[0] = V.bcur[1] = 0;
   if (l == 0) H.hook_left = 0;
   if (l == (int) H.lev.size () - 1) {
      if (H.coarse_inv) {
         if (H.coarse_invf) launch_dense_matvec_f32_batch (K, H.coarse_invf, H.coarse_ldf, V.bb, V.bx, (int) V.n, st);
         else launch_dense_matvec_batch (K, H.coarse_inv, V.bb, V.bx, (int) V.n, st);
         return;
      }
      const int sweeps = H.tune->ml_coarsest_sweeps > 0 ? H.tune->ml_coarsest_sweeps : 30;
      launch_fill (V.bx, 0.0, nk, st);
      column_solves_batch (H, V, K, 0, V.bb, V.bx, 0, st);
      launch_csr_spmv_batch (K, V.L, V.color_rb[1], V.color_rb[2], V.bx, V.br, V.bb, 1, st);
      column_solves_batch (H, V, K, 1, V.br, V.bx, 1, st);
      for (int s = 1; s < sweeps; s++)
         for (int step = 0; step < 2; step++) {
            const int c = (s & 1) ? 1 - step : step;
            launch_csr_spmv_batch (K, V.L, V.color_rb[c], V.color_rb[c + 1], V.bx, V.br, V.bb, 1, st);
            column_solves_batch (H, V, K, c, V.br, V.bx, 1, st);
         }
      return;
   }
   const int nu = (l >= H.coarse_from) ? H.nu_coarse : H.nu;
   if (l == 0 && H.hook) H.hook_left = 4 * nu;
   launch_fill (V.bx, 0.0, nk, st);
   if (V.wave_fused) {
      column_solves_batch (H, V, K, 0, V.bb, V.bx2, 0, st);
      V.bcur[0] = 1;
      after_half_sweep (H, V, 0, V.bx2, K, st);
      gs_half_batch (H, V, K, 1, st);
   } else {
      column_solves_batch (H, V, K, 0, V.bb, V.bx, 0, st);
      after_half_sweep (H, V, 0, V.bx, K, st);
      gs_half_batch (H, V, K, 1, st);
   }
   for (int s = 1; s < nu; s++) { gs_half_batch (H, V, K, 0, st); gs_half_batch (H, V, K, 1, st); }
   MlLevel &C = H.lev[l + 1];
   const int gamma = (l >= H.gamma_from && l < H.gamma_to) ? 2 : 1;
   for (int g = 0; g < gamma; g++) {
      launch_csr_spmv_batch (K, V.L, 0, V.L.nrowblk, V.bxnow (), V.br, V.bb, 1, st);
      launch_restrict_sum_batch (K, V.rptr, V.ridx, V.br, C.bb, V.nc, st);
      ml_cycle_batch (H, K, l + 1, st);
      launch_prolong_add_batch (K, V.cmap, C.bxnow (), V.bxnow (), V.n, H.omega, st);
   }
   for (int s = 0; s < nu; s++) { gs_half_batch (H, V, K, 1, st); gs_half_batch (H, V, K, 0, st); }
}

void ml_apply_batch (MlHierarchy &H, int K, const double *r, double *z, hipStream_t st)
{
   MlLevel &V = H.lev[0];
   launch_gather_batch (K, H.perm0, r, V.bb, V.n, st);
   ml_cycle_batch (H, K, 0, st);
   launch_scatter_batch (K, H.perm0, V.bxnow (), z, V.n, st);
}

void ml_apply_batch_split (MlHierarchy &H, int K, const double *const *src, double *z, double *const *dst, hipStream_t st, const double *src_scale)
{
   MlLevel &V = H.lev[0];
   launch_gather_interleave (K, H.perm0, src, V.bb, V.n, st, src_scale);
   ml_cycle_batch (H, K, 0, st);
   launch_scatter_split (K, H.perm0, V.bxnow (), z, dst, V.n, st);
}

void ml_apply_batch_split_ext (MlHierarchy &H, int K, const double *const *src, const double *halo, const int *sel, int64_t n_own, double *z,
                               double *const *dst, hipStream_t st, const MlSmoothHook *hook)
{
   MlLevel &V = H.lev[0];
   if (sel) launch_gather_interleave_ext (K, H.perm0, src, halo, sel, n_own, V.bb, V.n, st);
   else launch_gather_interleave_ext_block (K, H.perm0, src, halo, n_own, V.bb, V.n, st);
   H.hook = hook;
   ml_cycle_batch (H, K, 0, st);
   H.hook = nullptr;
   launch_scatter_split_own (K, H.perm0, V.bxnow (), z, dst, n_own, V.n, st);
}

void ml_time_piece (MlHierarchy &H, int which, hipStream_t st)
{
   MlLevel &V = H.lev[0];
   if (H.lev.size () < 2) return;
   if (which == 0) {
      if (V.L.dg_val) launch_diag_residual (V.L, V.color_tile[0], V.color_tile[1], V.x, V.b, V.r, st);
      else launch_csr_residual_range (V.L, V.color_rb[0], V.color_rb[1], V.x, V.b, V.r, st);
   }
   else launch_colblock_apply_lanes (V.B, V.color_grp[0], V.color_grp[1], V.r, V.x, 1, st);
}

int64_t ml_bytes (const MlHierarchy &H, int which)
{
   if (H.lev.size () < 2) return 0;
   auto level_piece = [&] (const MlLevel &V, int colour, int what) -> int64_t {
      const int64_t rows = colour == 0 ? V.rows0 : V.n - V.rows0;
      const int64_t vb = V.L.valf ? 4 : 8, fb = V.B.fac_tf ? 4 : 8;
      if (what == 0 && V.L.dg_val) {
         const double share = V.n ? (double) rows / (double) V.n : 0.0;
         return (int64_t) (share * ((double) V.L.dg_nval * 4.0 + (double) V.L.dg_ntile * (double) sizeof (DgTile) + (double) V.L.dg_ngrp * (double) sizeof (DgGroup))) + rows * (8 + 8) + V.n * 8;
      }
      if (what == 0) {
         const double per_row = V.n ? (double) V.L.nnz / (double) V.n : 0.0;
         return (int64_t) (per_row * (double) rows * (double) (vb + 4)) + rows * (4 + 8 + 8) + V.n * 8;
      }
      return rows * ((2 * V.B.P + 1) * fb + 8 + 8 + 8);
   };
   if (which == 0 || which == 1) return level_piece (H.lev[0], 0, which);
   int64_t total = 0;
   for (size_t l = 0; l + 1 < H.lev.size (); l++) {
      const MlLevel &V = H.lev[l];
      const int nu = ((int) l >= H.coarse_from) ? H.nu_coarse : H.nu;
      for (int c = 0; c < 2; c++) {
         total += (int64_t) (2 * nu) * level_piece (V, c, 1);
         total += (int64_t) (2 * nu - (c == 0 ? 1 : 0)) * level_piece (V, c, 0);
         if (V.lane_diag) {
            const int64_t rows = c == 0 ? V.rows0 : V.n - V.rows0, slots = (int64_t) (V.color_grp[c + 1] - V.color_grp[c]) * V.B.gw;
            total -= (int64_t) (2 * nu - (c == 0 ? 1 : 0)) * (rows * (8 + 8) - slots * 4);
         }
      }
      if (V.L.dg_val) total += V.L.dg_nval * 4 + (int64_t) V.L.dg_ntile * (int64_t) sizeof (DgTile) + (int64_t) V.L.dg_ngrp * (int64_t) sizeof (DgGroup) + V.n * (8 + 8 + 8);
      else total += V.L.nnz * ((V.L.valf ? 4 : 8) + 4) + V.n * (4 + 8 + 8 + 8);
      total += V.n * (8 + 4) + V.nc * (8 + 4);
      total += V.n * (8 + 8 + 4) + V.nc * 8;
   }
   const int64_t ncoarse = H.lev.back ().n;
   total += ncoarse * ncoarse * 8 + 2 * ncoarse * 8;
   total += H.lev[0].n * (8 + 8 + 4) * 2;
   return total;
}
```

nk_ocn_tracer_jacobian_precond_amd/csrc/multilevel.h:

```cpp
#pragma once
#include "nkp_dev.h"

#include <vector>

struct MlLevel {
   int64_t n = 0;
   CsrDev L;
   ColBlocksDev B;
   int color_rb[3] = { 0, 0, 0 };
   int color_blk[3] = { 0, 0, 0 };
   int color_grp[3] = { 0, 0, 0 };
   int color_tile[3] = { 0, 0, 0 };
   int64_t rows0 = 0;
   int wave_columns = 0;
   int wave_fused = 0;
   int wave_diag = 0;
   int lane_diag = 0;
   int64_t nc = 0;
   int *cmap = nullptr;
   int *rptr = nullptr, *ridx = nullptr;
   double *x = nullptr, *b = nullptr, *r = nullptr;
   double *x2 = nullptr;
   int cur[2] = { 0, 0 };
   double *bx = nullptr, *bx2 = nullptr, *bb = nullptr, *br = nullptr;
   int bcur[2] = { 0, 0 };
   double *bxbuf (int k) { return k ? bx2 : bx; }
   double *bxnow () { return bxbuf (bcur[0]); }
   std::vector<int> nat_inv;
   double *xbuf (int k) { return k ? x2 : x; }
   double *xnow () { return xbuf (cur[0]); }
};

struct MlSmoothHook {
   void (*refresh) (void *ctx, int colour, double *x, int K, hipStream_t st);
   void *ctx;
};

struct MlHierarchy {
   std::vector<MlLevel> lev;
   const MlSmoothHook *hook = nullptr;
   int hook_left = 0;
   int *perm0 = nullptr;
   double *coarse_inv = nullptr;
   float *coarse_invf = nullptr;
   int coarse_ldf = 0;
   int nu = 1;
   int nu_coarse = 1;
   int coarse_from = 2;
   int f32 = 1;
   int fused = 1;
   int tail_from = -1;
   int gamma_from = 0, gamma_to = 0;
   double omega = 1.1;
   const nkp_tuning *tune = nullptr;
   size_t device_bytes = 0;
   double setup_seconds = 0.0;
   int levels_on_device = 0;
   int inverse_pivoted = 0;
   int batch_K = 0;
   int default_build = 0;
};

inline bool ml_level_fused (const MlHierarchy &H, const MlLevel &V)
{
   const int fused_max = H.tune->ml_fused_max_cols;
   return V.wave_fused || V.lane_diag || (H.fused && V.B.gs_ok && (fused_max <= 0 || V.color_grp[2] * V.B.gw <= fused_max));
}

int ml_setup (MlHierarchy &H, int64_t n, const int *rowptr, const int *colind, const double *val,
              const int *blk_start, int64_t nblk, const int *col_i, const int *col_j, const int *col_t ,
              int tracer_cnt, int max_levels, int nu, int coarsest_rows, int verbose, int rank,
              hipStream_t st, char *err, size_t errlen, const nkp_tuning &tune, const CsrDev *A_dev = nullptr );
void ml_free (MlHierarchy &H);
int ml_coarse_inverse (const MlHierarchy &H, int n, const int *prow, const int *pcol, const double *pval, double **inv, float **invf,
                       int *ldf, size_t *bytes, hipStream_t st);
inline int ml_level0_sweeps (const MlHierarchy &H) { return 0 >= H.coarse_from ? H.nu_coarse : H.nu; }
inline bool ml_level0_hookable (const MlHierarchy &H) { return H.lev.size () >= 2 && H.tail_from != 0 && ml_level0_sweeps (H) > 0; }
void ml_apply (MlHierarchy &H, const double *r, double *z, hipStream_t st, const MlSmoothHook *hook = nullptr);
int ml_batch_prepare (MlHierarchy &H, int K);
void ml_apply_batch (MlHierarchy &H, int K, const double *r, double *z, hipStream_t st);
void ml_apply_batch_split (MlHierarchy &H, int K, const double *const *src, double *z, double *const *dst, hipStream_t st, const double *src_scale = nullptr);
void ml_apply_batch_split_ext (MlHierarchy &H, int K, const double *const *src, const double *halo, const int *sel, int64_t n_own, double *z,
                               double *const *dst, hipStream_t st, const MlSmoothHook *hook = nullptr);
void ml_time_piece (MlHierarchy &H, int which, hipStream_t st);
int64_t ml_bytes (const MlHierarchy &H, int which);
int ml_tail_launch (MlHierarchy &H, int l0, hipStream_t st);
```

nk_ocn_tracer_jacobian_precond_amd/csrc/nkp_dev.h:

```cpp
#pragma once
#include <hip/hip_runtime.h>
#include <stdint.h>

#include "../../include/nkp.h"
#include "col_plan.h"
#include "tuning.h"

#include <type_traits>
#include <utility>
#include <vector>

#define NKP_WAVE 64
#define NKP_MAX_K 512
#define NKP_SPMV_LDS_NNZ 2048
#define NKP_SPMV_MAX_ROWS 256

struct alignas (16) DgTile {
   int row0, rows;
   int kl0, len;
   int k0, nk;
   int g0, ng;
   long long voff;
};
struct DgGroup {
   int key0;
   int slots;
};
#define DG_RUN_MAX 5

struct CsrDev {
   int64_t n = 0, nnz = 0;
   int *rowptr = nullptr;
   int *colind = nullptr;
   double *val = nullptr;
   float *valf = nullptr;
   int *rowblk = nullptr;
   int nrowblk = 0;
   unsigned short *codes = nullptr;
   int *dict = nullptr;
   int *dict_ptr = nullptr;
   int *dg_ptr = nullptr;
   int *dg_key = nullptr;
   long long *dg_voff = nullptr;
   float *dg_val = nullptr;
   double *dg_vald = nullptr;
   DgTile *dg_tile = nullptr;
   int *dg_gptr = nullptr;
   DgGroup *dg_grp = nullptr;
   int dg_ntile = 0, dg_ncol = 0, dg_nkey = 0, dg_ngrp = 0;
   int64_t dg_nval = 0;
   const nkp_tuning *tune = nullptr;
};

double build_spmv_codes_host (int64_t n, const int *rowptr, const int *colind, const int *rowblk, int nrowblk,
                              unsigned short **codes_out, int **dict_out, int *ndict_out, int **dict_ptr_out);
int attach_spmv_codes (CsrDev &A, const int *h_rowptr, const int *h_colind, const int *h_rowblk, size_t *device_bytes);

void launch_csr_spmv (const CsrDev &A, const double *x, double *y, const double *b, int mode, hipStream_t st);
void launch_csr_residual_range (const CsrDev &A, int rb0, int rb1, const double *x, const double *b, double *y, hipStream_t st);
void launch_csr_spmv_range (const CsrDev &A, int rb0, int rb1, const double *x, double *y, const double *b, int mode, hipStream_t st);
void launch_csr_abs_spmv (const CsrDev &A, const double *x, const double *b, double *y, hipStream_t st);
int diag_build (CsrDev &L, const int *h_blk_start, const int *d_blk_start, int ncol, int ncol0, int max_len, int cap, int color_tile[3],
                size_t *device_bytes, hipStream_t st);
void launch_diag_fill (const CsrDev &L, hipStream_t st);
void launch_diag_residual (const CsrDev &L, int tile0, int tile1, const double *x, const double *b, double *y, hipStream_t st);
void launch_diag_spmv (const CsrDev &A, const double *x, double *y, const double *b, int mode, hipStream_t st);
void build_rowblocks_host (int64_t n, const int *rowptr, int **rowblk_out, int *nrowblk_out);

void launch_value_gradient (int K, int nk, const CsrDev &A, const double *lam, const double *x, double alpha, int accumulate, double *g, hipStream_t st);
void launch_values_product (int K, int nk, const CsrDev &A, const double *val, const double *x, double alpha, int accumulate, double *y, int64_t ldy, hipStream_t st);

struct ColBlocksDev {
   int64_t n = 0;
   int nblk = 0;
   int *blk_start = nullptr;
   int P = 0;
   int max_len = 0;
   int dropped = 0;
   double *fac = nullptr;
   int ngrp = 0;
   int *grp_b0 = nullptr;
   int *grp_nb = nullptr;
   int *grp_maxlen = nullptr;
   long long *grp_base = nullptr;
   int *grp_row0 = nullptr;
   int *col_slot = nullptr;
   double *fac_t = nullptr;
   float *fac_tf = nullptr;
   int lds_doubles = 0;
   int gw = 64;
   int rhs_slots = 0;
   int stream = 0;
   int ldsres = 0;
   int gs_ok = 0;
   int gs_lds_bytes = 0;
   int *gs_rb_ptr = nullptr;
   int *gs_rb = nullptr;
   int *wave_desc = nullptr;
   int *grp_tile = nullptr;
   int grp_tile_cnt = 0;
   const nkp_tuning *tune = nullptr;
   int ml_level = 0;
   ColKernel kern;
   std::vector<int> *grp_cols = nullptr;
};


template <int V> using int_tag = std::integral_constant<int, V>;
template <int V0, int... Vs, class F>
inline auto with_int (int v, F &&f)
{
   if constexpr (sizeof... (Vs) == 0) return f (int_tag<V0> ());
   else {
      if (v == V0) return f (int_tag<V0> ());
      return with_int<Vs...> (v, f);
   }
}
template <class F> inline auto with_band (int P, F &&f) { return with_int<1, 2, 4> (P, f); }
template <class F> inline auto with_k (int K, F &&f) { return with_int<2, 4, 8> (K, f); }
template <class F> inline auto with_bool (bool b, F &&f) { return b ? f (std::true_type ()) : f (std::false_type ()); }
template <class F> inline auto with_storage (const float *vf, const double *vd, F &&f) { return vf ? f (vf) : f (vd); }
template <class PTR> using elem_t = std::remove_cv_t<std::remove_pointer_t<PTR>>;
template <class F>
inline auto with_band_rows (const ColBlocksDev &B, F &&f)
{
   return with_band (B.P, [&] (auto p) { return with_int<1, 2> (B.max_len <= NKP_WAVE ? 1 : 2, [&] (auto rpl) { return f (p, rpl); }); });
}

template <int... Is, class F>
__device__ __forceinline__ void static_for_seq (std::integer_sequence<int, Is...>, F &&f) { (f (int_tag<Is> ()), ...); }
template <int N, class F>
__device__ __forceinline__ void static_for (F &&f) { static_for_seq (std::make_integer_sequence<int, N> (), f); }

template <int LANE>
__device__ __forceinline__ double readlane_const_f64 (double v)
{
   int lo = __double2loint (v), hi = __double2hiint (v);
   lo = __builtin_amdgcn_readlane (lo, LANE);
   hi = __builtin_amdgcn_readlane (hi, LANE);
   return __hiloint2double (hi, lo);
}

template <int P, int RPL, int K>
__device__ __forceinline__ void wave_band_sweeps (int len, int lane, double (&y)[RPL][K], const double (&invd)[RPL], const double (&L)[RPL][P],
                                                  const double (&U)[RPL][P])
{
   constexpr int ROWS = RPL * NKP_WAVE;
   len = __builtin_amdgcn_readfirstlane (len);
   double bc[K];
#pragma unroll
   for (int j = 0; j < K; j++) bc[j] = readlane_const_f64<0> (y[0][j]);
   static_for<ROWS - 1> ([&] (auto kc) __attribute__ ((always_inline)) {
      constexpr int k = decltype (kc)::value;
      if (__builtin_expect (k < len - 1, 1)) {
         constexpr int s1 = (k + 1) / NKP_WAVE, l1 = (k + 1) % NKP_WAVE;
         double t[K], nb[K];
#pragma unroll
         for (int j = 0; j < K; j++) {
            t[j] = y[s1][j] - L[s1][0] * bc[j];
            nb[j] = readlane_const_f64<l1> (t[j]);
         }
#pragma unroll
         for (int j = 0; j < K; j++) y[s1][j] = lane == l1 ? t[j] : y[s1][j];
#pragma unroll
         for (int q = 2; q <= P; q++)
            if (k + q < ROWS) {
               const int s = (k + q) / NKP_WAVE, l = (k + q) % NKP_WAVE;
#pragma unroll
               for (int j = 0; j < K; j++) {
                  const double u = y[s][j] - L[s][q - 1] * bc[j];
                  y[s][j] = lane == l ? u : y[s][j];
               }
            }
#pragma unroll
         for (int j = 0; j < K; j++) bc[j] = nb[j];
      }
   });
   asm volatile ("" : "+s" (len));
   double c[K];
#pragma unroll
   for (int j = 0; j < K; j++) {
      c[j] = y[0][j];
      if (RPL == 2 && len > NKP_WAVE) c[j] = y[RPL - 1][j];
   }
   static_for<ROWS> ([&] (auto ic) __attribute__ ((always_inline)) {
      constexpr int k = ROWS - 1 - decltype (ic)::value;
      if (__builtin_expect (k < len, 1)) {
         constexpr int s0 = k / NKP_WAVE, l0 = k % NKP_WAVE;
         double v[K];
#pragma unroll
         for (int j = 0; j < K; j++) {
            v[j] = c[j] * invd[s0];
            bc[j] = readlane_const_f64<l0> (v[j]);
         }
         if (k > 0) {
            constexpr int s1 = (k > 0 ? k - 1 : 0) / NKP_WAVE;
#pragma unroll
            for (int j = 0; j < K; j++) c[j] = y[s1][j] - U[s1][0] * bc[j];
         }
#pragma unroll
         for (int j = 0; j < K; j++) y[s0][j] = lane == l0 ? v[j] : y[s0][j];
#pragma unroll
         for (int q = 2; q <= P; q++)
            if (k - q >= 0) {
               const int s = (k - q) / NKP_WAVE, l = (k - q) % NKP_WAVE;
#pragma unroll
               for (int j = 0; j < K; j++) {
                  const double u = y[s][j] - U[s][q - 1] * bc[j];
                  y[s][j] = lane == l ? u : y[s][j];
               }
            }
      }
   });
}

int colblock_build_lane_layout (ColBlocksDev &B, const int *h_blk_start, const int *ranges, int nranges,
                                int *grp_first, size_t *device_bytes, hipStream_t st, int f32 = 0, const int *h_rowptr = nullptr);
int colblock_repack_lane_layout (const ColBlocksDev &B, const int *d_gcols, hipStream_t st);
int launch_gs_fused (const CsrDev &L, const ColBlocksDev &B, int g0, int g1, const double *xa, const double *xb, int split,
                     const double *b, double *xout, hipStream_t st);
void launch_colblock_apply_lanes (const ColBlocksDev &B, int g0, int g1, const double *r, double *z, int accumulate, hipStream_t st);

void launch_colblock_measure (const CsrDev &A, const ColBlocksDev &B, int *d_out2 , hipStream_t st);
void launch_colblock_factor (const CsrDev &A, ColBlocksDev &B, int *d_status, hipStream_t st);
void launch_colblock_apply (const ColBlocksDev &B, const double *r, double *z, hipStream_t st);
void launch_colblock_apply_range (const ColBlocksDev &B, int b0, int b1, const double *r, double *z, int accumulate, hipStream_t st);
void launch_colblock_apply_range_r32 (const ColBlocksDev &B, int b0, int b1, const double *r, double *z, int accumulate, hipStream_t st);
void launch_build_wave_desc (const CsrDev &L, ColBlocksDev &B, hipStream_t st);
void launch_gs_wave (const CsrDev &L, const ColBlocksDev &B, int b0, int b1, const double *xa, const double *xb, int split, const double *b, double *xout,
                     int r32, hipStream_t st);
void launch_gs_wave_diag (const CsrDev &L, const ColBlocksDev &B, int tile0, int tile1, const double *xa, const double *xb, int split, const double *b,
                          double *xout, int r32, hipStream_t st);
void launch_gs_lanes_diag (const CsrDev &L, const ColBlocksDev &B, int g0, int g1, const double *xa, const double *xb, int split, const double *b,
                           double *xout, hipStream_t st);

#define NKP_BATCH_MAX 8
#define NKP_RED_BLOCKS 1024
#define NKP_DOT_CHUNK 8

void launch_multi_dot (const void *V, int v_f32, int64_t ld, int k, const double *w, int64_t n, double *partial, double *out, hipStream_t st);
void launch_update_w (const void *V, int v_f32, int64_t ld, int k, const double *h, double *w, int64_t n, double *partial, double *out_nrm2, hipStream_t st);
void launch_scale_to (const double *x, const double *alpha_dev, double *y, float *yf, int64_t n, hipStream_t st);
void launch_axpy_multi (const double *Z, int64_t ld, int k, const double *c, double *x, int64_t n, hipStream_t st);
void launch_dot (const double *x, const double *y, int64_t n, double *partial, double *out, hipStream_t st);
void launch_berr (const double *r, const double *den, int64_t n, double *partial, double *out, hipStream_t st);
void launch_count_entries (const double *x, int64_t n, double *partial, double *out, hipStream_t st);
void launch_finish_column (double *h, const double *h2, int k, const double *nrm2, double *inv, hipStream_t st);
void launch_finish_column_pythagoras (double *h, int k, double *inv, hipStream_t st);
struct GsGroup {
   const double *V[NKP_BATCH_MAX];
   double *w[NKP_BATCH_MAX];
   double *partial[NKP_BATCH_MAX];
   double *vnext[NKP_BATCH_MAX];
};
void launch_multi_dot_group (int R, const GsGroup &G, int64_t ld, int k, int64_t n, double *msg, hipStream_t st);
void launch_update_w_group (int R, const GsGroup &G, int64_t ld, int k, const double *msg, int64_t n, double *nrm2, hipStream_t st);
void launch_finish_column_group (int R, double *msg, const double *msg2, int k, const double *nrm2, double *inv, hipStream_t st);
void launch_scale_to_group (int R, const GsGroup &G, const double *inv, int64_t n, hipStream_t st);
void launch_axpby (double a, const double *x, double b, double *y, int64_t n, hipStream_t st);
void launch_copy (const double *x, double *y, int64_t n, hipStream_t st);
void launch_vmul (const double *x, const double *w, double *y, int64_t n, hipStream_t st);
void launch_fill (double *y, double v, int64_t n, hipStream_t st);

void launch_restrict_sum (const int *rptr, const int *ridx, const double *fine, double *coarse, int64_t nc, hipStream_t st);
void launch_prolong_add (const int *cmap, const double *coarse, double *fine, int64_t nf, double omega, hipStream_t st);
void launch_gather (const int *perm, const double *in, double *out, int64_t n, hipStream_t st);
void launch_scatter (const int *perm, const double *in, double *out, int64_t n, hipStream_t st);
void launch_dense_matvec (const double *Minv, const double *x, double *y, int n, hipStream_t st);
void launch_dense_matvec_f32 (const float *Minv, int ld, const double *x, double *y, int n, hipStream_t st);
void launch_dense_matvec_f32_batch (int K, const float *Minv, int ld, const double *x, double *y, int n, hipStream_t st);
int dense_inverse_blocked_device (int n, const int *h_rowptr, const int *h_col, const double *h_val, double **inv_out, float **invf_out, int *ldf_out,
                                  size_t *bytes, hipStream_t st);
bool dense_inverse_device (int n, const std::vector<double> &host_a, double **inv_out, size_t *bytes, hipStream_t st);

void launch_interleave (int K, const double *const *src , double *X, int64_t n, hipStream_t st, const double *scale = nullptr);
void launch_deinterleave (int K, const double *X, double *const *dst , int64_t n, hipStream_t st);
void launch_csr_spmv_batch (int K, const CsrDev &A, int rb0, int rb1, const double *x, double *y, const double *b, int mode, hipStream_t st,
                            const double *scale = nullptr );
void launch_restrict_sum_batch (int K, const int *rptr, const int *ridx, const double *fine, double *coarse, int64_t nc, hipStream_t st);
void launch_prolong_add_batch (int K, const int *cmap, const double *coarse, double *fine, int64_t nf, double omega, hipStream_t st);
void launch_gather_batch (int K, const int *perm, const double *in, double *out, int64_t n, hipStream_t st);
void launch_scatter_batch (int K, const int *perm, const double *in, double *out, int64_t n, hipStream_t st);
void launch_gather_interleave (int K, const int *perm, const double *const *src, double *out, int64_t n, hipStream_t st, const double *scale = nullptr);
void launch_scatter_split (int K, const int *perm, const double *in, double *z, double *const *dst, int64_t n, hipStream_t st);
void launch_csr_spmv_batch_split (int K, const CsrDev &A, const double *x, double *const *dst, hipStream_t st, const double *scale = nullptr);
void launch_csr_spmv_batch_split_range (int K, const CsrDev &A, int rb0, int rb1, const double *x, double *const *dst, hipStream_t st, const double *scale = nullptr);
void launch_csr_residual_batch_split_range (int K, const CsrDev &A, int rb0, int rb1, const double *x, const double *const *b, const double *bscale,
                                            double *const *dst, hipStream_t st);
void launch_add_split (int K, const double *p, double *z, double *const *dst, int64_t n, hipStream_t st);
void launch_pack_rows_split (int K, const int *idx, const double *const *src, double *out, int64_t nrows, hipStream_t st);
void launch_gather_interleave_ext (int K, const int *perm, const double *const *src, const double *halo, const int *sel, int64_t n_own, double *out, int64_t n,
                                   hipStream_t st);
void launch_gather_interleave_ext_block (int K, const int *perm, const double *const *src, const double *recv, int64_t n_own, double *out, int64_t n, hipStream_t st);
void launch_scatter_split_own (int K, const int *perm, const double *in, double *z, double *const *dst, int64_t n_own, int64_t n, hipStream_t st);
void launch_dense_matvec_batch (int K, const double *Minv, const double *x, double *y, int n, hipStream_t st);
void launch_colblock_apply_wave_batch (int K, const ColBlocksDev &B, int b0, int b1, const double *r, double *z, int accumulate, int r32, hipStream_t st);
void launch_gs_wave_batch (int K, const CsrDev &L, const ColBlocksDev &B, int b0, int b1, const double *xa, const double *xb, int split, const double *b, double *xout,
                           int r32, hipStream_t st);
int launch_colblock_apply_lanes_batch (int K, const ColBlocksDev &B, int g0, int g1, const double *r, double *z, int accumulate, hipStream_t st);
```

nk_ocn_tracer_jacobian_precond_amd/csrc/solver_impl.h:

```cpp
#pragma once
#include "../../include/nkp.h"
#include "nkp_dev.h"
#include "multilevel.h"
#include "refactor.h"
#include "dist_plan.h"
#include "krylov_host.h"

#include <atomic>
#include <initializer_list>
#include <memory>
#include <string>
#include <vector>

#define HIPCHK(call)                                                                             \
   do {                                                                                          \
      hipError_t e_ = (call);                                                                    \
      if (e_ != hipSuccess) return fail (NKP_EDEVICE, "%s failed: %s (%s:%d)", #call, hipGetErrorString (e_), __FILE__, __LINE__); \
   } while (0)

struct nkp_solver {
   nkp_options opt;
   nkp_tuning tune;
   int device = 0;
   bool stagnated = false;
   int rhs_class = 0;
   bool borrowed = false;
   hipStream_t stream = nullptr;
   bool own_stream = false;
   CsrDev A;
   ColBlocksDev B;
   MlHierarchy ml;
   struct {
      bool on = false;
      nkp_comm_ops ops;
      int64_t n_global = 0, fst = 0, n_halo = 0, nsend = 0;
      std::vector<int> send_counts, recv_counts;
      int *send_idx = nullptr;
      double *sendbuf = nullptr;
      double *xe = nullptr;
      int seg_rb[4] = { 0, 0, 0, 0 };
      bool overlap = false;
      hipStream_t comm_stream = nullptr;
      hipEvent_t ev_packed = nullptr, ev_halo = nullptr;
      bool ras = false;
      int64_t n_ext = 0, n_sel = 0;
      int *sel_idx = nullptr;
      double *rext = nullptr, *zext = nullptr;
      int ras_rings = 0;
      bool ras_sep = false;
      int64_t ras_nsend = 0;
      int *ras_send_idx = nullptr;
      double *ras_sendbuf = nullptr, *bras_send = nullptr, *bras_recv = nullptr;
      std::vector<int> ras_send_counts, ras_recv_counts, ras_send_counts_k, ras_recv_counts_k;
      bool smooth = false;
      MlSmoothHook smooth_hook = { nullptr, nullptr };
      std::vector<int32_t> h_smooth_send[2], h_smooth_recv[2];
      int *smooth_send_idx[2] = { nullptr, nullptr }, *smooth_recv_idx[2] = { nullptr, nullptr };
      std::vector<int> smooth_send_counts[2], smooth_recv_counts[2], smooth_send_counts_k[2], smooth_recv_counts_k[2];
      int64_t smooth_nsend_max = 0, smooth_nrecv_max = 0;
      double *smooth_sendbuf = nullptr, *smooth_recvbuf = nullptr, *bsmooth_send = nullptr, *bsmooth_recv = nullptr;
      double *bxe = nullptr, *bsend = nullptr, *gmsg = nullptr, *ghpin = nullptr;
      int bK = 0;
      int agreed_K = 0;
      std::vector<int> send_counts_k, recv_counts_k;
      std::vector<int64_t> starts;
      std::vector<int32_t> h_halo_rows, h_send_rows, own_blk, own_ci, own_cj, own_ct;
      bool own_has_blk = false;
      int own_tracer_cnt = 1;
   } dist;
   int64_t n = 0, ld = 0;
   int m = 0;
   bool vf32 = false;
   double *vcur = nullptr;
   double *V = nullptr, *Z = nullptr, *w = nullptr, *r = nullptr, *x = nullptr, *b = nullptr, *t1 = nullptr, *t2 = nullptr;
   double *p1 = nullptr, *p2 = nullptr;
   int precond_steps = 1;
   int steps_now = 1;
   bool equil = false;
   double *rscale = nullptr, *rinv = nullptr;
   double *eqtmp = nullptr;
   bool comm_failed = false;
   double *partial = nullptr;
   double *dscal = nullptr;
   double *hpin = nullptr;
   int *dint = nullptr;
   std::vector<nkp_solver *> batch_members;
   double *bvin = nullptr, *bz = nullptr, *bw = nullptr;
   int batch_K = 0;
   int64_t batch_steps = 0;
   int batch_width = 0;
   size_t device_bytes = 0;
   double create_seconds = 0.0;
   struct Shared {
      std::atomic<int> clones { 0 };
      std::atomic<int64_t> alltoallv_calls { 0 }, allreduce_calls { 0 };
      bool broken = false;
      std::string why;
   };
   std::shared_ptr<Shared> shared = std::make_shared<Shared> ();
   RefactorWork *rf = nullptr;
   std::vector<int> h_blk, h_col_i, h_col_j, h_col_t;
   int tracer_cnt = 1;
   int64_t refactor_count = 0;
   int refactor_rebuilt = 0;
   double refactor_seconds = 0.0;
   DistRefactorPlan *dplan = nullptr;
   int64_t refactor_halo_values = 0;
   nkp_solver *trans = nullptr, *trans_of = nullptr;
   int *trans_src = nullptr;
   double *trans_val = nullptr;
   size_t trans_map_bytes = 0;
   double trans_seconds = 0.0, trans_kernel_seconds = 0.0;
   int *trans_ship = nullptr;
   double *trans_send = nullptr, *trans_recv = nullptr;
   std::vector<int> trans_send_counts, trans_recv_counts;
   int64_t trans_nnz = 0, trans_sent = 0, trans_received = 0;
   struct {
      double *lam = nullptr, *x = nullptr, *stage = nullptr, *g = nullptr;
      size_t lam_cap = 0, x_cap = 0, stage_cap = 0, g_cap = 0;
      int64_t calls = 0;
      double seconds = 0.0;
   } vg;
   struct {
      double *x = nullptr, *stage = nullptr, *r = nullptr;
      size_t x_cap = 0, stage_cap = 0, r_cap = 0;
      int64_t calls = 0, tangent_calls = 0;
      double seconds = 0.0;
   } vp;
   double *h_dev () { return dscal; }
   double *h2_dev () { return dscal + (m + 2); }
   double *misc_dev () { return dscal + 2 * (m + 2); }
   double *y_dev () { return dscal + 2 * (m + 2) + 16; }
};

template <class T>
static int dev_alloc (nkp_solver *s, T **p, size_t count)
{
   void *q = nullptr;
   size_t bytes = (count ? count : 1) * sizeof (T);
   hipError_t e = hipMalloc (&q, bytes);
   if (e != hipSuccess) return fail (NKP_ENOMEM, "hipMalloc of %zu bytes failed: %s", bytes, hipGetErrorString (e));
   *p = (T *) q;
   s->device_bytes += bytes;
   return NKP_OK;
}


struct Want {
   double **p;
   size_t *cap;
   size_t need;
};

inline int reserve (nkp_solver *s, std::initializer_list<Want> set, const char *who)
{
   double *fresh[8] = {};
   int rc = NKP_OK;
   size_t i = 0;
   for (const Want &w : set) {
      if (w.need > *w.cap) {
         void *q = nullptr;
         if (hipMalloc (&q, w.need * sizeof (double)) != hipSuccess) {
            rc = fail (NKP_ENOMEM, "%s: hipMalloc of %zu bytes of work space failed", who, w.need * sizeof (double));
            break;
         }
         fresh[i] = (double *) q;
      }
      i++;
   }
   if (rc) {
      for (double *q : fresh)
         if (q) (void) hipFree (q);
      (void) hipGetLastError ();
      return rc;
   }
   i = 0;
   for (const Want &w : set) {
      if (fresh[i]) {
         if (*w.p) {
            (void) hipFree (*w.p);
            s->device_bytes -= *w.cap * sizeof (double);
         }
         *w.p = fresh[i];
         *w.cap = w.need;
         s->device_bytes += w.need * sizeof (double);
      }
      i++;
   }
   return NKP_OK;
}

inline int width_of (int nrhs) { return nrhs <= 1 ? 1 : nrhs <= 2 ? 2 : nrhs <= 4 ? 4 : 8; }

inline void alltoallv_dev (nkp_solver *s, const double *send, const int *send_counts, double *recv, const int *recv_counts, hipStream_t st)
{
   s->shared->alltoallv_calls++;
   if (s->dist.ops.alltoallv (s->dist.ops.ctx, send, send_counts, recv, recv_counts, (void *) st)) s->comm_failed = true;
}

inline void allreduce_dev (nkp_solver *s, double *dev, int count, int op)
{
   if (!s->dist.on) return;
   s->shared->allreduce_calls++;
   if (s->dist.ops.allreduce (s->dist.ops.ctx, dev, count, op, (void *) s->stream)) s->comm_failed = true;
}

inline int refactor_broken (const nkp_solver *s) { return fail (NKP_ESINGULAR, "%s", s->shared->why.c_str ()); }

inline int sev_of (int c) { return c == NKP_OK ? 0 : c == NKP_OK_BERR ? 1 : c == NKP_NOT_CONVERGED ? 2 : 3; }

#define NKP_BERR_ROUNDING_LEVEL 1.0e-14

NKP_PRIVATE void solver_free (nkp_solver *s);
NKP_PRIVATE void msg (const nkp_solver *s, int lvl, const char *fmt, ...);
struct SpmvMatrixHost {
   int64_t nnz, ncols;
   const int32_t *rowptr, *colind;
   const double *val;
};
struct PrecondMatrixHost {
   int64_t n, nblk;
   const int32_t *rowptr, *colind;
   const double *val;
   const int32_t *blk_start, *col_i, *col_j, *col_t;
};
NKP_PRIVATE int create_impl (nkp_solver **out, const nkp_options *opt_in, int64_t n, int64_t nnz,
                             const int32_t *rowptr, const int32_t *colind, const double *val,
                             const int32_t *blk_start, int64_t nblk, int coupled_tracer_cnt, const SpmvMatrixHost *spmv_mat,
                             const PrecondMatrixHost *pm = nullptr);
NKP_PRIVATE int clone_impl (nkp_solver *src, nkp_solver **out, bool member);
NKP_PRIVATE void drop_intertracer (int64_t n, int tracer_cnt, const int32_t *rowptr, const int32_t *colind, const double *val,
                                   std::vector<int32_t> &f_rowptr, std::vector<int32_t> &f_colind, std::vector<double> &f_val);
NKP_PRIVATE void apply_precond_once (nkp_solver *s, const double *rin, double *zout);
NKP_PRIVATE void apply_precond (nkp_solver *s, const double *rin, double *zout);
NKP_PRIVATE void spmv_op (nkp_solver *s, const double *x, double *y, const double *b, int mode);
NKP_PRIVATE void arnoldi_apply (nkp_solver *s, int j);
NKP_PRIVATE void arnoldi_orthogonalise (nkp_solver *s, int j);
NKP_PRIVATE void arnoldi_step_device (nkp_solver *s, int j);
NKP_PRIVATE int fg_begin (nkp_solver *s, FgmresState &F);
NKP_PRIVATE int fg_restart (nkp_solver *s, FgmresState &F);
NKP_PRIVATE bool fg_post_step (nkp_solver *s, FgmresState &F);
NKP_PRIVATE int fg_end_cycle (nkp_solver *s, FgmresState &F);
NKP_PRIVATE int rhs_refused (int verdict, const char *what);
NKP_PRIVATE int backward_error (nkp_solver *s, double *berr);
NKP_PRIVATE const char *batch_unsupported (const nkp_solver *s);
NKP_PRIVATE void note_fallback (const nkp_solver *s, const char *who, const char *why, int nrhs);
NKP_PRIVATE int batch_prepare_exchange (nkp_solver *s, int K);
NKP_PRIVATE int dist_agree (nkp_solver *s, int local_rc, const char *who, const char *where);
NKP_PRIVATE bool smooth_install (nkp_solver *s, const DistPlan &D);
NKP_PRIVATE int smooth_build_lists (nkp_solver *s);
NKP_PRIVATE const MlSmoothHook *smooth_hook_of (nkp_solver *s);
NKP_PRIVATE void smooth_release (nkp_solver *s);
NKP_PRIVATE void launch_smooth_pack (int K, const int *idx, const double *x, double *out, int64_t nrows, hipStream_t st);
NKP_PRIVATE void launch_smooth_unpack (int K, const int *idx, const double *in, double *x, int64_t nrows, hipStream_t st);
NKP_PRIVATE void valgrad_release (nkp_solver *s);
NKP_PRIVATE int valgrad_time_prepare (nkp_solver *s, int K);
NKP_PRIVATE void valgrad_time_launch (nkp_solver *s, int K);
NKP_PRIVATE int fetch_x_operand (nkp_solver *s, int K, const double *const *xp, double *il, const double **x_in, const char *who);
NKP_PRIVATE void valprod_release (nkp_solver *s);
NKP_PRIVATE int valprod_time_prepare (nkp_solver *s, int K, int which);
NKP_PRIVATE void valprod_time_launch (nkp_solver *s, int K);
NKP_PRIVATE void valprod_time_composition (nkp_solver *s, int K);
NKP_PRIVATE void trans_release (nkp_solver *s);
NKP_PRIVATE void trans_detach (nkp_solver *t);
NKP_PRIVATE void trans_set_stream (nkp_solver *s);
NKP_PRIVATE int64_t trans_device_bytes (const nkp_solver *s);
NKP_PRIVATE int trans_gather_values (nkp_solver *s, const double **d_valT);
NKP_PRIVATE int trans_dist_follow (nkp_solver *s, int flags, const char *who, int (*refactor) (nkp_solver *t, const void *d_val, int flags, const char *who));
```

nk_ocn_tracer_jacobian_precond_amd/csrc/tuning.cpp:

```cpp
#include "tuning.h"

#include <stdarg.h>
#include <stdio.h>
#include <stdlib.h>
#include <string.h>

static thread_local std::string g_last_error;

int fail (int code, const char *fmt, ...)
{
   char buf[512];
   va_list ap;
   va_start (ap, fmt);
   vsnprintf (buf, sizeof buf, fmt, ap);
   va_end (ap);
   g_last_error = buf;
   return code;
}

extern "C" const char *nkp_last_error (void) { return g_last_error.c_str (); }
std::string last_error_message () { return g_last_error; }
void restore_error_message (const std::string &text) { g_last_error = text; }

extern "C" int nkp_default_options (nkp_options *opt)
{
   if (!opt) return NKP_EINVAL;
   memset (opt, 0, sizeof *opt);
   opt->struct_size = (int) sizeof (nkp_options);
   opt->precond = NKP_PRECOND_MULTILEVEL;
   opt->krylov = NKP_KRYLOV_FGMRES;
   opt->restart = 200;
   opt->max_iters = 20000;
   opt->rtol = 1.0e-10;
   opt->atol = 0.0;
   opt->device = -1;
   opt->verbose = 0;
   opt->rank = 0;
   opt->reorth = 0;
   opt->ml_levels = 0;
   opt->ml_smooth = 3;
   opt->precond_steps = 0;
   opt->equil = 0;
   opt->basis_f32 = 0;
   return NKP_OK;
}

static void builtin_tuning (nkp_tuning *t)
{
   memset (t, 0, sizeof *t);
   t->struct_size = (int) sizeof (nkp_tuning);
   t->ml_split = 1; t->ml_pocket = 4; t->ml_big_from = -3; t->ml_coarsest_rows = 8000; t->ml_dense_max = 8192;
   t->ml_theta = 0.0; t->ml_tau = 0.01; t->ml_device_min = 100000;
   t->ml_smooth_coarse = 0; t->ml_coarse_from = 2; t->ml_gamma_from = 0; t->ml_gamma_to = 0; t->ml_f32 = 1; t->ml_host_inverse = 0;
   t->ml_fused = 0; t->ml_fused_max_cols = 0; t->ml_wave_fused = 1; t->ml_coarsest_sweeps = 30; t->ml_tail_rows = 0; t->ml_omega = 1.1;
   t->col_ldsres = 2; t->col_stream = 1; t->col_stream_min = -1; t->col_stream_gw = 32; t->col_wave_max = 8192; t->col_w3 = 1;
   t->col_group = 8; t->col_pipe_min = 0; t->col_ldsres_early = 0; t->col_ldsres_packed = 1; t->col_sort_groups = 1;
   t->spmv_variant = 4; t->spmv_compress = 0; t->spmv_pipe_min = 1024; t->spmv_run = 1; t->spmv_wgs = 256;
   t->rhs_batch = 1; t->batch_spmv_rows = 1; t->precond_steps = 0; t->equil = -1; t->dist_overlap = 1; t->dist_ras = 1; t->dist_one_reduce = 0; t->force_dist = 0; t->setup_threads = 0; t->plan_times = 0;
   t->ml_drop_intertracer = 0; t->ml_huge_from = -1; t->dist_ras_rings = 1; t->ml_diag = 32; t->spmv_diag = 32;
   t->ml_lane_fused = 50000; t->dist_smooth_exchange = 0;
}

const nkp_tuning &nkp_builtin_tuning ()
{
   static const nkp_tuning t = [] { nkp_tuning q; builtin_tuning (&q); return q; } ();
   return t;
}

extern "C" int nkp_default_tuning (nkp_tuning *t)
{
   if (!t) return NKP_EINVAL;
   builtin_tuning (t);
   const char *e;
#define ENV_INT(name, field) do { if ((e = getenv (name)) && *e) t->field = atoi (e); } while (0)
#define ENV_POS(name, field) do { if ((e = getenv (name)) && atoi (e) > 0) t->field = atoi (e); } while (0)
#define ENV_FLAG(name, field) do { if ((e = getenv (name)) && *e) t->field = atoi (e) != 0; } while (0)
   ENV_FLAG ("NKP_ML_SPLIT", ml_split); ENV_INT ("NKP_ML_POCKET", ml_pocket); ENV_INT ("NKP_ML_BIG_FROM", ml_big_from);
   ENV_INT ("NKP_ML_COARSEST_ROWS", ml_coarsest_rows); ENV_INT ("NKP_ML_DENSE_MAX", ml_dense_max);
   if ((e = getenv ("NKP_ML_THETA")) && *e) t->ml_theta = atof (e);
   if ((e = getenv ("NKP_ML_TAU")) && *e) t->ml_tau = atof (e);
   if ((e = getenv ("NKP_ML_DEVICE_MIN")) && *e) t->ml_device_min = atoll (e);
   ENV_POS ("NKP_ML_SMOOTH_COARSE", ml_smooth_coarse); ENV_POS ("NKP_ML_COARSE_FROM", ml_coarse_from);
   ENV_INT ("NKP_ML_GAMMA_FROM", ml_gamma_from); ENV_INT ("NKP_ML_GAMMA_TO", ml_gamma_to);
   ENV_FLAG ("NKP_ML_F32", ml_f32); ENV_FLAG ("NKP_ML_HOST_INVERSE", ml_host_inverse); ENV_FLAG ("NKP_ML_FUSED", ml_fused);
   ENV_INT ("NKP_ML_FUSED_MAX_COLS", ml_fused_max_cols); ENV_INT ("NKP_ML_WAVE_FUSED", ml_wave_fused); ENV_POS ("NKP_ML_COARSEST_SWEEPS", ml_coarsest_sweeps);
   if ((e = getenv ("NKP_ML_TAIL_ROWS")) && *e) t->ml_tail_rows = atoll (e);
   if ((e = getenv ("NKP_ML_OMEGA")) && atof (e) > 0.0) t->ml_omega = atof (e);
   ENV_INT ("NKP_COL_LDSRES", col_ldsres); ENV_FLAG ("NKP_COLSTREAM", col_stream); ENV_INT ("NKP_COLSTREAM_MIN", col_stream_min);
   if ((e = getenv ("NKP_COLSTREAM_GW")) && *e) t->col_stream_gw = atoi (e) == 64 ? 64 : 32;
   ENV_INT ("NKP_COLWAVE_MAX", col_wave_max); ENV_FLAG ("NKP_COL_W3", col_w3); ENV_INT ("NKP_COLGROUP", col_group);
   ENV_INT ("NKP_COLPIPE_MIN", col_pipe_min); ENV_FLAG ("NKP_LDSRES_EARLY", col_ldsres_early); ENV_FLAG ("NKP_COL_PACKED", col_ldsres_packed); ENV_FLAG ("NKP_COL_SORT_GROUPS", col_sort_groups); ENV_INT ("NKP_COL_LDSRES_MIN", col_ldsres_min); ENV_INT ("NKP_ML_HUGE_FROM", ml_huge_from);
   ENV_INT ("NKP_SPMV_VARIANT", spmv_variant); ENV_FLAG ("NKP_SPMV_COMPRESS", spmv_compress); ENV_INT ("NKP_SPMV_PIPE_MIN", spmv_pipe_min);
   ENV_POS ("NKP_SPMV_RUN", spmv_run); ENV_POS ("NKP_SPMV_WGS", spmv_wgs);
   ENV_INT ("NKP_RHS_BATCH", rhs_batch); ENV_FLAG ("NKP_BATCH_SPMV_ROWS", batch_spmv_rows);
   ENV_POS ("NKP_PRECOND_STEPS", precond_steps); ENV_FLAG ("NKP_EQUIL", equil);
   ENV_FLAG ("NKP_DIST_OVERLAP", dist_overlap); ENV_FLAG ("NKP_DIST_RAS", dist_ras); ENV_FLAG ("NKP_DIST_ONE_REDUCE", dist_one_reduce);
   if (getenv ("NKP_FORCE_DIST")) t->force_dist = 1;
   ENV_POS ("NKP_SETUP_THREADS", setup_threads);
   if (getenv ("NKP_ML_PLAN_TIMES")) t->plan_times = 1;
   ENV_FLAG ("NKP_ML_DROP_INTERTRACER", ml_drop_intertracer);
   ENV_INT ("NKP_DIST_RAS_RINGS", dist_ras_rings);
   ENV_INT ("NKP_ML_DIAG", ml_diag);
   ENV_INT ("NKP_SPMV_DIAG", spmv_diag);
   ENV_INT ("NKP_ML_LANE_FUSED", ml_lane_fused);
   ENV_INT ("NKP_DIST_SMOOTH_EXCHANGE", dist_smooth_exchange);
#undef ENV_INT
#undef ENV_POS
#undef ENV_FLAG
   if (t->spmv_variant < 0 || t->spmv_variant > 9) t->spmv_variant = 4;
   return NKP_OK;
}

int resolve_tuning (const nkp_options *opt, nkp_tuning *out, bool *range_error)
{
   if (range_error) *range_error = false;
   if (opt && opt->tuning) {
      if (opt->tuning->struct_size != (int) sizeof (nkp_tuning)) return fail (NKP_EINVAL, "nkp_tuning.struct_size mismatch (%d != %zu)", opt->tuning->struct_size, sizeof (nkp_tuning));
      *out = *opt->tuning;
   } else {
      const int rc = nkp_default_tuning (out);
      if (rc) return rc;
   }
   if (out->dist_ras_rings < 0 || out->dist_ras_rings > 4) {
      if (range_error) *range_error = true;
      return fail (NKP_EINVAL, "nkp_tuning.dist_ras_rings = %d is out of range (0 = default, 1 .. 4 rings)", out->dist_ras_rings);
   }
   if (out->dist_smooth_exchange != 0 && out->dist_smooth_exchange != 1) {
      if (range_error) *range_error = true;
      return fail (NKP_EINVAL, "nkp_tuning.dist_smooth_exchange = %d is out of range (0 = off, 1 = on)", out->dist_smooth_exchange);
   }
   return NKP_OK;
}
```

nk_ocn_tracer_jacobian_precond_amd/solver.py:

```python
from __future__ import annotations

import ctypes as C
import os

import numpy as np

_HERE = os.path.dirname(os.path.abspath(__file__))
HIP_LIB_PATH = os.path.join(_HERE, "csrc", "libnkp_hip.so")
HOST_LIB_PATH = os.path.join(_HERE, "host", "libnkp_host.so")

PRECOND_NONE, PRECOND_COLUMN_JACOBI, PRECOND_MULTILEVEL = 0, 1, 3
KRYLOV_FGMRES, KRYLOV_BICGSTAB = 0, 1
NKP_OK, NKP_NOT_CONVERGED, NKP_BREAKDOWN, NKP_OK_BERR = 0, 1, 2, 3
REFACTOR_REBUILD = 1

ABI_SYMBOLS = [
    "nkp_default_options", "nkp_device_count", "nkp_create", "nkp_solve", "nkp_solve_device",
    "nkp_spmv", "nkp_spmv_device", "nkp_precond_apply", "nkp_multi_dot", "nkp_time_kernel",
    "nkp_get_int", "nkp_set_stream", "nkp_destroy", "nkp_last_error", "nkp_comm_unique_id",
    "nkp_comm_rccl_init", "nkp_comm_rccl_free", "nkp_create_dist", "nkp_dist_plan_host", "nkp_set_device",
    "nkp_gather_root", "nkp_clone", "nkp_ml_plan_host", "nkp_comm_file_init", "nkp_comm_file_free",
    "nkp_create64", "nkp_cell_major_order", "nkp_permuted_rows", "nkp_dist_overlap_plan_host", "nkp_dist_plan_size",
    "nkp_dist_plan_copy", "nkp_dist_plan_free", "nkp_ml_level_array", "nkp_default_tuning", "nkp_solve_batch_device",
    "nkp_refactor", "nkp_refactor_device", "nkp_refactor_dist", "nkp_refactor_dist_device", "nkp_transpose", "nkp_transpose_dist",
    "nkp_value_gradient", "nkp_value_gradient_device",
    "nkp_values_product", "nkp_values_product_device", "nkp_solve_tangent_device", "nkp_matrix_array",
]

_ALLREDUCE_FN = C.CFUNCTYPE(C.c_int, C.c_void_p, C.c_void_p, C.c_int, C.c_int, C.c_void_p)
_ALLTOALLV_FN = C.CFUNCTYPE(C.c_int, C.c_void_p, C.c_void_p, C.POINTER(C.c_int), C.c_void_p, C.POINTER(C.c_int), C.c_void_p)
_ALLTOALLV_I32_FN = C.CFUNCTYPE(C.c_int, C.c_void_p, C.POINTER(C.c_int32), C.POINTER(C.c_int), C.POINTER(C.c_int32), C.POINTER(C.c_int))
_ALLGATHER_I64_FN = C.CFUNCTYPE(C.c_int, C.c_void_p, C.c_int64, C.POINTER(C.c_int64))


class NkpCommOps(C.Structure):
    _fields_ = [("ctx", C.c_void_p), ("rank", C.c_int), ("nranks", C.c_int), ("allreduce", _ALLREDUCE_FN),
                ("alltoallv", _ALLTOALLV_FN), ("alltoallv_i32_host", _ALLTOALLV_I32_FN),
                ("allgather_i64_host", _ALLGATHER_I64_FN)]


class NkpTuning(C.Structure):
    _fields_ = [
        ("struct_size", C.c_int), ("ml_split", C.c_int), ("ml_pocket", C.c_int), ("ml_big_from", C.c_int), ("ml_coarsest_rows", C.c_int),
        ("ml_dense_max", C.c_int), ("ml_theta", C.c_double), ("ml_tau", C.c_double), ("ml_device_min", C.c_int64),
        ("ml_smooth_coarse", C.c_int), ("ml_coarse_from", C.c_int), ("ml_gamma_from", C.c_int), ("ml_gamma_to", C.c_int), ("ml_f32", C.c_int),
        ("ml_host_inverse", C.c_int), ("ml_fused", C.c_int), ("ml_fused_max_cols", C.c_int), ("ml_wave_fused", C.c_int), ("ml_coarsest_sweeps", C.c_int),
        ("ml_tail_rows", C.c_int64), ("ml_omega", C.c_double),
        ("col_ldsres", C.c_int), ("col_stream", C.c_int), ("col_stream_min", C.c_int), ("col_stream_gw", C.c_int), ("col_wave_max", C.c_int),
        ("col_w3", C.c_int), ("col_group", C.c_int), ("col_pipe_min", C.c_int), ("col_ldsres_early", C.c_int), ("col_ldsres_packed", C.c_int),
        ("spmv_variant", C.c_int), ("spmv_compress", C.c_int), ("spmv_pipe_min", C.c_int), ("spmv_run", C.c_int), ("spmv_wgs", C.c_int),
        ("rhs_batch", C.c_int), ("precond_steps", C.c_int), ("equil", C.c_int), ("dist_overlap", C.c_int), ("dist_ras", C.c_int), ("force_dist", C.c_int),
        ("setup_threads", C.c_int), ("plan_times", C.c_int), ("ml_drop_intertracer", C.c_int), ("dist_one_reduce", C.c_int), ("ml_huge_from", C.c_int), ("col_ldsres_min", C.c_int), ("col_sort_groups", C.c_int), ("batch_spmv_rows", C.c_int),
        ("dist_ras_rings", C.c_int), ("ml_diag", C.c_int), ("spmv_diag", C.c_int), ("ml_lane_fused", C.c_int),
        ("dist_smooth_exchange", C.c_int),
    ]


class NkpOptions(C.Structure):
    _fields_ = [
        ("struct_size", C.c_int), ("precond", C.c_int), ("krylov", C.c_int), ("restart", C.c_int),
        ("max_iters", C.c_int), ("rtol", C.c_double), ("atol", C.c_double), ("device", C.c_int),
        ("verbose", C.c_int), ("rank", C.c_int), ("reorth", C.c_int), ("ml_levels", C.c_int),
        ("ml_smooth", C.c_int), ("basis_f32", C.c_int), ("precond_steps", C.c_int), ("equil", C.c_int), ("reserved", C.c_int * 4),
        ("col_i", C.POINTER(C.c_int32)), ("col_j", C.POINTER(C.c_int32)), ("col_t", C.POINTER(C.c_int32)),
        ("tuning", C.POINTER(NkpTuning)),
    ]


class NkpError(RuntimeError):
    def __init__(self, code, message):
        super().__init__(f"nkp error {code}: {message}")
        self.code = code


_lib = None


def load_library(path=None):
    global _lib
    if _lib is not None and path is None:
        return _lib
    path = path or HIP_LIB_PATH
    if not os.path.exists(path):
        raise FileNotFoundError(
            f"{path} not found: build it with `python -c 'import __graft_entry__ as g; g.build()'` "
            "(there is no CPU fallback for the solve path)")
    lib = C.CDLL(path, mode=C.RTLD_GLOBAL)
    i32p, f64p, vp = C.POINTER(C.c_int32), C.POINTER(C.c_double), C.c_void_p
    lib.nkp_default_options.argtypes = [C.POINTER(NkpOptions)]
    lib.nkp_device_count.restype = C.c_int
    lib.nkp_create.argtypes = [C.POINTER(vp), C.POINTER(NkpOptions), C.c_int64, C.c_int64, i32p, i32p, f64p, i32p, C.c_int64, C.c_int]
    lib.nkp_create64.argtypes = [C.POINTER(vp), C.POINTER(NkpOptions), C.c_int64, C.POINTER(C.c_int64), i32p, f64p, i32p, C.c_int64, C.c_int]
    lib.nkp_solve.argtypes = [vp, f64p, C.c_int, C.c_int64, f64p, C.POINTER(C.c_int), f64p]
    lib.nkp_solve_device.argtypes = [vp, vp, vp, C.c_int, f64p, C.POINTER(C.c_int), f64p]
    lib.nkp_solve_batch_device.argtypes = [vp, C.c_int, vp, vp, C.c_int64, f64p, C.POINTER(C.c_int), f64p]
    lib.nkp_spmv.argtypes = [vp, f64p, f64p]
    lib.nkp_spmv_device.argtypes = [vp, vp, vp]
    lib.nkp_precond_apply.argtypes = [vp, f64p, f64p]
    lib.nkp_multi_dot.argtypes = [vp, f64p, C.c_int64, C.c_int, f64p, f64p]
    lib.nkp_time_kernel.argtypes = [vp, C.c_int, C.c_int, C.c_int, f64p]
    lib.nkp_get_int.argtypes = [vp, C.c_char_p]
    lib.nkp_get_int.restype = C.c_int64
    lib.nkp_ml_level_array.argtypes = [vp, C.c_int, C.c_char_p, vp, C.c_int64]
    lib.nkp_ml_level_array.restype = C.c_int64
    lib.nkp_matrix_array.argtypes = [vp, C.c_char_p, vp, C.c_int64]
    lib.nkp_matrix_array.restype = C.c_int64
    lib.nkp_set_stream.argtypes = [vp, vp]
    lib.nkp_destroy.argtypes = [vp]
    lib.nkp_destroy.restype = None
    lib.nkp_last_error.restype = C.c_char_p
    lib.nkp_comm_unique_id.argtypes = [vp]
    lib.nkp_comm_rccl_init.argtypes = [C.POINTER(NkpCommOps), vp, C.c_int, C.c_int]
    lib.nkp_comm_rccl_free.argtypes = [C.POINTER(NkpCommOps)]
    lib.nkp_comm_rccl_free.restype = None
    lib.nkp_create_dist.argtypes = [C.POINTER(vp), C.POINTER(NkpOptions), C.c_int64, C.c_int64, C.c_int64, C.c_int64,
                                    i32p, i32p, f64p, i32p, C.c_int64, C.c_int, C.POINTER(NkpCommOps)]
    lib.nkp_set_device.argtypes = [C.c_int]
    lib.nkp_gather_root.argtypes = [vp, f64p, f64p]
    lib.nkp_clone.argtypes = [vp, C.POINTER(vp)]
    lib.nkp_transpose.argtypes = [vp, C.POINTER(vp)]
    lib.nkp_transpose_dist.argtypes = [vp, C.POINTER(vp)]
    lib.nkp_value_gradient.argtypes = [vp, C.c_int, f64p, f64p, C.c_int64, C.c_double, C.c_int, f64p]
    lib.nkp_value_gradient_device.argtypes = [vp, C.c_int, vp, vp, C.c_int64, C.c_double, C.c_int, vp]
    lib.nkp_values_product.argtypes = [vp, C.c_int, f64p, f64p, C.c_int64, C.c_double, C.c_int, f64p, C.c_int64]
    lib.nkp_values_product_device.argtypes = [vp, C.c_int, vp, vp, C.c_int64, C.c_double, C.c_int, vp, C.c_int64]
    lib.nkp_solve_tangent_device.argtypes = [vp, C.c_int, vp, vp, C.c_int64, vp, vp, C.c_int64, f64p, C.POINTER(C.c_int), f64p]
    lib.nkp_refactor.argtypes = [vp, f64p, C.c_int]
    lib.nkp_refactor_device.argtypes = [vp, vp, C.c_int]
    lib.nkp_refactor_dist.argtypes = [vp, f64p, C.c_int]
    lib.nkp_refactor_dist_device.argtypes = [vp, vp, C.c_int]
    lib.nkp_dist_plan_host.argtypes = [C.c_int64, C.c_int64, i32p, i32p, C.c_int, C.c_int, C.POINTER(C.c_int64), i32p, i32p,
                                       C.POINTER(C.c_int64), i32p]
    lib.nkp_ml_plan_host.argtypes = [C.c_int64, i32p, i32p, f64p, i32p, C.c_int64, i32p, i32p, C.c_int, C.c_int, C.c_int, C.c_int64,
                                     C.POINTER(C.c_int), C.POINTER(C.c_int64), i32p, i32p]
    if path == HIP_LIB_PATH:
        _lib = lib
    return lib


def ml_plan_host(rowptr, colind, val, blk_start, col_i=None, col_j=None, coupled_tracer_cnt=1, max_levels=0, coarsest_rows=8000):
    lib = load_library()
    rowptr = np.ascontiguousarray(rowptr, np.int32)
    colind = np.ascontiguousarray(colind, np.int32)
    val = np.ascontiguousarray(val, np.float64)
    blk_start = np.ascontiguousarray(blk_start, np.int32)
    n = rowptr.size - 1
    ip = lambda a: None if a is None else _p(np.ascontiguousarray(a, np.int32), C.c_int32)
    ci = None if col_i is None else np.ascontiguousarray(col_i, np.int32)
    cj = None if col_j is None else np.ascontiguousarray(col_j, np.int32)
    cap = 2 * n + 64
    cmap, colof = np.empty(cap, np.int32), np.empty(cap, np.int32)
    rows = np.zeros(64, np.int64)
    nlev = C.c_int()
    rc = lib.nkp_ml_plan_host(n, _p(rowptr, C.c_int32), _p(colind, C.c_int32), _p(val, C.c_double), _p(blk_start, C.c_int32), blk_start.size - 1,
                              None if ci is None else _p(ci, C.c_int32), None if cj is None else _p(cj, C.c_int32), coupled_tracer_cnt, max_levels,
                              coarsest_rows, cap, C.byref(nlev), _p(rows, C.c_int64), _p(cmap, C.c_int32), _p(colof, C.c_int32))
    if rc != 0:
        raise NkpError(rc, "nkp_ml_plan_host failed")
    rows = rows[:nlev.value]
    cmaps, colofs, qc, qo = [], [], 0, 0
    for l in range(nlev.value - 1):
        cmaps.append(cmap[qc:qc + rows[l]].copy())
        colofs.append(colof[qo:qo + rows[l + 1]].copy())
        qc += rows[l]
        qo += rows[l + 1]
    return rows, cmaps, colofs


def default_options(**overrides):
    lib = load_library()
    o = NkpOptions()
    lib.nkp_default_options(C.byref(o))
    for k, v in overrides.items():
        if not hasattr(o, k):
            raise AttributeError(f"nkp_options has no field {k}")
        setattr(o, k, v)
    return o


def default_tuning(**overrides):
    lib = load_library()
    t = NkpTuning()
    lib.nkp_default_tuning.argtypes = [C.POINTER(NkpTuning)]
    lib.nkp_default_tuning(C.byref(t))
    for k, v in overrides.items():
        if not hasattr(t, k):
            raise AttributeError(f"nkp_tuning has no field {k}")
        setattr(t, k, v)
    return t


def _p(a, t):
    return a.ctypes.data_as(C.POINTER(t))


def cell_major_order(blk_start, coupled_tracer_cnt):
    lib = load_library()
    blk = np.ascontiguousarray(blk_start, np.int32)
    nblk, n = blk.size - 1, int(blk[-1])
    perm = np.empty(max(n, 1), np.int32)
    blk_new = np.empty(nblk + 1, np.int32)
    col_t = np.empty(max(nblk, 1), np.int32)
    col_src = np.empty(max(nblk, 1), np.int32)
    lib.nkp_cell_major_order.argtypes = [C.c_int64, C.POINTER(C.c_int32), C.c_int] + [C.POINTER(C.c_int32)] * 4
    rc = lib.nkp_cell_major_order(nblk, _p(blk, C.c_int32), int(coupled_tracer_cnt), _p(perm, C.c_int32), _p(blk_new, C.c_int32),
                                  _p(col_t, C.c_int32), _p(col_src, C.c_int32))
    if rc != 0:
        raise NkpError(rc, lib.nkp_last_error().decode())
    perm = perm[:n]
    inv = np.empty(n, np.int32)
    inv[perm] = np.arange(n, dtype=np.int32)
    return perm, inv, blk_new, col_t[:nblk], col_src[:nblk]


def permuted_rows(rowptr, colind, val, perm, inv, r0, r1):
    lib = load_library()
    rowptr = np.ascontiguousarray(rowptr, np.int32)
    colind = np.ascontiguousarray(colind, np.int32)
    val = np.ascontiguousarray(val, np.float64)
    perm = np.ascontiguousarray(perm, np.int32)
    inv = np.ascontiguousarray(inv, np.int32)
    old = perm[r0:r1]
    nloc = int((rowptr[old.astype(np.int64) + 1].astype(np.int64) - rowptr[old]).sum())
    rp = np.empty(r1 - r0 + 1, np.int32)
    ci = np.empty(max(nloc, 1), np.int32)
    v = np.empty(max(nloc, 1), np.float64)
    lib.nkp_permuted_rows.argtypes = [C.c_int64, C.POINTER(C.c_int32), C.POINTER(C.c_int32), C.POINTER(C.c_double), C.POINTER(C.c_int32),
                                      C.POINTER(C.c_int32), C.c_int64, C.c_int64, C.POINTER(C.c_int32), C.POINTER(C.c_int32), C.POINTER(C.c_double)]
    rc = lib.nkp_permuted_rows(rowptr.size - 1, _p(rowptr, C.c_int32), _p(colind, C.c_int32), _p(val, C.c_double), _p(perm, C.c_int32),
                               _p(inv, C.c_int32), int(r0), int(r1), _p(rp, C.c_int32), _p(ci, C.c_int32), _p(v, C.c_double))
    if rc != 0:
        raise NkpError(rc, lib.nkp_last_error().decode())
    return rp, ci[:nloc], v[:nloc]


class NkpSolver:

    def __init__(self, rowptr, colind, val, blk_start=None, coupled_tracer_cnt=1, col_i=None, col_j=None, col_t=None, **options):
        self._lib = load_library()
        self._h = C.c_void_p()
        self._rowptr64 = np.ascontiguousarray(rowptr, np.int64) if np.asarray(rowptr).dtype == np.int64 else None
        rowptr = np.ascontiguousarray(rowptr, np.int32) if self._rowptr64 is None else self._rowptr64
        colind = np.ascontiguousarray(colind, np.int32)
        val = np.ascontiguousarray(val, np.float64)
        self.n = int(rowptr.size - 1)
        self.nnz = int(colind.size)
        tuning = options.pop("tuning", None)
        opt = default_options(**options)
        self.options = opt
        if tuning is not None:
            self._tuning = tuning if isinstance(tuning, NkpTuning) else default_tuning(**tuning)
            opt.tuning = C.pointer(self._tuning)
        if col_i is not None and col_j is not None:
            col_i = np.ascontiguousarray(col_i, np.int32)
            col_j = np.ascontiguousarray(col_j, np.int32)
            if blk_start is None or col_i.size != len(blk_start) - 1 or col_j.size != col_i.size:
                raise ValueError("col_i / col_j need one entry per block of blk_start")
            opt.col_i, opt.col_j = _p(col_i, C.c_int32), _p(col_j, C.c_int32)
        if col_t is not None:
            col_t = np.ascontiguousarray(col_t, np.int32)
            if blk_start is None or col_t.size != len(blk_start) - 1:
                raise ValueError("col_t needs one entry per block of blk_start")
            opt.col_t = _p(col_t, C.c_int32)
        if blk_start is not None:
            blk_start = np.ascontiguousarray(blk_start, np.int32)
            bp, nb = _p(blk_start, C.c_int32), blk_start.size - 1
        else:
            bp, nb = None, 0
        if self._rowptr64 is not None:
            rc = self._lib.nkp_create64(C.byref(self._h), C.byref(opt), self.n, _p(self._rowptr64, C.c_int64),
                                        _p(colind, C.c_int32), _p(val, C.c_double), bp, nb, coupled_tracer_cnt)
        else:
            rc = self._lib.nkp_create(C.byref(self._h), C.byref(opt), self.n, self.nnz, _p(rowptr, C.c_int32),
                                      _p(colind, C.c_int32), _p(val, C.c_double), bp, nb, coupled_tracer_cnt)
        if rc != 0:
            self._h = C.c_void_p()
            raise NkpError(rc, self._lib.nkp_last_error().decode())

    @classmethod
    def _from_handle(cls, lib, handle, n, nnz, options):
        self = cls.__new__(cls)
        self._lib, self._h, self.n, self.nnz, self.options = lib, handle, n, nnz, options
        return self

    def _check(self, rc, allow=(0,)):
        if rc not in allow:
            raise NkpError(rc, self._lib.nkp_last_error().decode())
        return rc

    def solve(self, b, raise_on_fail=True):
        x = np.array(b, np.float64, order="C", copy=True).reshape(-1)
        if x.size != self.n:
            raise ValueError(f"b has {x.size} entries, expected {self.n}")
        berr, relres, iters = C.c_double(), C.c_double(), C.c_int()
        rc = self._lib.nkp_solve(self._h, _p(x, C.c_double), 1, self.n, C.byref(berr), C.byref(iters), C.byref(relres))
        self._check(rc, (0,) if raise_on_fail else (0, 1, 2, 3))
        return x, dict(status=rc, iters=iters.value, relres=relres.value, berr=berr.value)

    def solve_device(self, d_b, d_x, use_guess=False, raise_on_fail=True):
        berr, relres, iters = C.c_double(), C.c_double(), C.c_int()
        rc = self._lib.nkp_solve_device(self._h, C.c_void_p(d_b), C.c_void_p(d_x), int(use_guess), C.byref(berr),
                                        C.byref(iters), C.byref(relres))
        self._check(rc, (0,) if raise_on_fail else (0, 1, 2, 3))
        return dict(status=rc, iters=iters.value, relres=relres.value, berr=berr.value)

    def solve_batch_device(self, d_B, d_X, nrhs, ldb, raise_on_fail=True):
        berr, relres, iters = (C.c_double * nrhs)(), (C.c_double * nrhs)(), (C.c_int * nrhs)()
        rc = self._lib.nkp_solve_batch_device(self._h, nrhs, C.c_void_p(d_B), C.c_void_p(d_X), ldb, berr, iters, relres)
        self._check(rc, (0,) if raise_on_fail else (0, 1, 2, 3))
        return [dict(status=rc, iters=iters[c], relres=relres[c], berr=berr[c]) for c in range(nrhs)]

    def solve_many(self, B, raise_on_fail=True):
        X = np.array(B, np.float64, order="C", copy=True)
        nrhs = X.shape[0]
        berr, relres, iters = (C.c_double * nrhs)(), (C.c_double * nrhs)(), (C.c_int * nrhs)()
        rc = self._lib.nkp_solve(self._h, _p(X, C.c_double), nrhs, X.shape[1], berr, iters, relres)
        self._check(rc, (0,) if raise_on_fail else (0, 1, 2, 3))
        return X, [dict(status=rc, iters=iters[c], relres=relres[c], berr=berr[c]) for c in range(nrhs)]

    def refactor(self, val, rebuild=False):
        val = np.ascontiguousarray(val, np.float64).reshape(-1)
        if val.size != self.nnz:
            raise ValueError(f"val has {val.size} entries, expected {self.nnz}")
        self._check(self._lib.nkp_refactor(self._h, _p(val, C.c_double), REFACTOR_REBUILD if rebuild else 0))

    def refactor_device(self, d_val, rebuild=False):
        self._check(self._lib.nkp_refactor_device(self._h, C.c_void_p(d_val), REFACTOR_REBUILD if rebuild else 0))

    def value_gradient(self, lam, x, alpha=-1.0):
        lam = np.ascontiguousarray(np.atleast_2d(np.asarray(lam, np.float64)))
        x = np.ascontiguousarray(np.atleast_2d(np.asarray(x, np.float64)))
        if lam.ndim != 2 or lam.shape != x.shape or lam.shape[1] != self.n:
            raise ValueError(f"lam and x must both have shape ({self.n},) or (K, {self.n})")
        g = np.empty(max(self.nnz, 1), np.float64)
        self._check_collective(self._lib.nkp_value_gradient(self._h, lam.shape[0], _p(lam, C.c_double), _p(x, C.c_double), self.n, float(alpha), 0,
                                                            _p(g, C.c_double)))
        return g[:self.nnz]

    def value_gradient_device(self, d_lam, d_x, nrhs, ld, d_g, alpha=-1.0, accumulate=False):
        self._check_collective(self._lib.nkp_value_gradient_device(self._h, int(nrhs), C.c_void_p(d_lam), C.c_void_p(d_x), int(ld), float(alpha),
                                                                   int(bool(accumulate)), C.c_void_p(d_g)))

    def values_product(self, val, X, alpha=1.0, Y=None):
        val = np.ascontiguousarray(val, np.float64).reshape(-1)
        x = np.ascontiguousarray(np.atleast_2d(np.asarray(X, np.float64)))
        if val.size != self.nnz or x.ndim != 2 or x.shape[1] != self.n:
            raise ValueError(f"val must hold {self.nnz} values and X have shape ({self.n},) or (K, {self.n})")
        if Y is None:
            y, acc = np.empty_like(x), 0
        else:
            y, acc = np.array(np.atleast_2d(np.asarray(Y, np.float64)), order="C", copy=True), 1
            if y.shape != x.shape:
                raise ValueError("Y must have the shape of X")
        v = val if val.size else np.zeros(1)
        self._check_collective(self._lib.nkp_values_product(self._h, x.shape[0], _p(v, C.c_double), _p(x, C.c_double), self.n, float(alpha), acc,
                                                            _p(y, C.c_double), self.n))
        return y.reshape(np.shape(X))

    def values_product_device(self, d_val, d_x, nrhs, ldx, d_y, ldy, alpha=1.0, accumulate=False):
        self._check_collective(self._lib.nkp_values_product_device(self._h, int(nrhs), C.c_void_p(d_val), C.c_void_p(d_x), int(ldx), float(alpha),
                                                                   int(bool(accumulate)), C.c_void_p(d_y), int(ldy)))

    def solve_tangent_device(self, d_dval, d_x, ldx, d_db, d_dx, nrhs, ld, raise_on_fail=True):
        berr, relres, iters = (C.c_double * nrhs)(), (C.c_double * nrhs)(), (C.c_int * nrhs)()
        rc = self._lib.nkp_solve_tangent_device(self._h, int(nrhs), C.c_void_p(d_dval or None), C.c_void_p(d_x or None), int(ldx), C.c_void_p(d_db or None),
                                                C.c_void_p(d_dx), int(ld), berr, iters, relres)
        self._check(rc, (0,) if raise_on_fail else (0, 1, 2, 3))
        return [dict(status=rc, iters=iters[c], relres=relres[c], berr=berr[c]) for c in range(nrhs)]

    def solve_tangent(self, X, dval=None, dB=None, raise_on_fail=True):
        if dval is None and dB is None:
            raise ValueError("solve_tangent needs dval or dB")
        x = np.ascontiguousarray(np.atleast_2d(np.asarray(X, np.float64)))
        K, n = x.shape
        if n != self.n:
            raise ValueError(f"X must have shape ({self.n},) or (K, {self.n})")
        bufs = []
        try:
            d_x = _device_array(bufs, x) if dval is not None else None
            d_v = _device_array(bufs, np.ascontiguousarray(dval, np.float64).reshape(-1), self.nnz) if dval is not None else None
            d_b = _device_array(bufs, np.ascontiguousarray(np.atleast_2d(np.asarray(dB, np.float64))), K * n) if dB is not None else None
            out = np.empty((K, n))
            d_o = _device_array(bufs, out)
            infos = self.solve_tangent_device(d_v, d_x, n, d_b, d_o, K, n, raise_on_fail)
            if out.nbytes:
                _hip_check(_hip().hipMemcpy(C.c_void_p(out.ctypes.data), C.c_void_p(d_o), C.c_size_t(out.nbytes), 2))
        finally:
            for q in bufs:
                _hip().hipFree(C.c_void_p(q))
        return out.reshape(np.shape(X)), infos

    def _check_collective(self, rc):
        self._check(rc)

    def spmv(self, x):
        x = np.ascontiguousarray(x, np.float64)
        y = np.empty(self.n)
        self._check(self._lib.nkp_spmv(self._h, _p(x, C.c_double), _p(y, C.c_double)))
        return y

    def spmv_device(self, d_x, d_y):
        self._check(self._lib.nkp_spmv_device(self._h, C.c_void_p(d_x), C.c_void_p(d_y)))

    def precond_apply(self, r):
        r = np.ascontiguousarray(r, np.float64)
        z = np.empty(self.n)
        self._check(self._lib.nkp_precond_apply(self._h, _p(r, C.c_double), _p(z, C.c_double)))
        return z

    def multi_dot(self, V, w):
        V = np.ascontiguousarray(V, np.float64)
        w = np.ascontiguousarray(w, np.float64)
        k = V.shape[0]
        out = np.empty(k + 1)
        self._check(self._lib.nkp_multi_dot(self._h, _p(V, C.c_double), V.shape[1], k, _p(w, C.c_double), _p(out, C.c_double)))
        return out

    def time_kernel(self, which, reps=20, arg=0):
        ms = C.c_double()
        self._check(self._lib.nkp_time_kernel(self._h, which, arg, reps, C.byref(ms)))
        return ms.value

    def get_int(self, key):
        return int(self._lib.nkp_get_int(self._h, key.encode()))

    _ML_ARRAY_TYPES = {"valf": np.float32, "val": np.float64, "fac": np.float64, "coarse_inv": np.float64, "color_blk": np.int32,
                       "col_kernel": np.int32, "dg_ptr": np.int32, "dg_key": np.int32, "dg_voff": np.int64, "dg_val": np.float32,
                       "dg_gptr": np.int32, "dg_grp": np.int32}

    def ml_level_array(self, level, what):
        cnt = int(self._lib.nkp_ml_level_array(self._h, level, what.encode(), None, 0))
        if cnt < 0:
            raise NkpError(cnt, last_error())
        out = np.empty(cnt, self._ML_ARRAY_TYPES.get(what, np.int32))
        if cnt:
            got = int(self._lib.nkp_ml_level_array(self._h, level, what.encode(), out.ctypes.data_as(C.c_void_p), out.nbytes))
            if got != cnt:
                raise NkpError(got, last_error())
        return out

    def matrix_array(self, what):
        cnt = int(self._lib.nkp_matrix_array(self._h, what.encode(), None, 0))
        if cnt < 0:
            raise NkpError(cnt, last_error())
        out = np.empty(cnt, {"dg_voff": np.int64, "dg_val": np.float64, "val": np.float64, "fac": np.float64}.get(what, np.int32))
        if cnt:
            got = int(self._lib.nkp_matrix_array(self._h, what.encode(), out.ctypes.data_as(C.c_void_p), out.nbytes))
            if got != cnt:
                raise NkpError(got, last_error())
        return out

    def set_stream(self, stream_ptr):
        self._check(self._lib.nkp_set_stream(self._h, C.c_void_p(stream_ptr)))

    def clone(self):
        h = C.c_void_p()
        self._check(self._lib.nkp_clone(self._h, C.byref(h)))
        c = object.__new__(NkpSolver)
        c._lib, c._h, c.n, c.nnz, c.options, c._parent = self._lib, h, self.n, self.nnz, self.options, self
        return c

    def transposed(self):
        h = C.c_void_p()
        self._check(self._lib.nkp_transpose(self._h, C.byref(h)))
        t = getattr(self, "_trans", None)
        if t is not None and t._h.value == h.value:
            return t
        t = object.__new__(NkpSolver)
        t._lib, t._h, t.n, t.nnz, t.options, t._parent, t._trans_of = self._lib, h, self.n, self.nnz, self.options, self, self
        self._trans = t
        return t

    def close(self):
        if getattr(self, "_h", None) and self._h.value:
            t = getattr(self, "_trans", None)
            if t is not None:
                t._h = C.c_void_p()
                self._trans = None
            owner = getattr(self, "_trans_of", None)
            if owner is not None and getattr(owner, "_trans", None) is self:
                owner._trans = None
            self._lib.nkp_destroy(self._h)
            self._h = C.c_void_p()

    def __del__(self):
        try:
            self.close()
        except Exception:
            pass

    def __enter__(self):
        return self

    def __exit__(self, *a):
        self.close()


_HIP = None


def _hip():
    global _HIP
    if _HIP is None:
        _HIP = C.CDLL("libamdhip64.so")
    return _HIP


def _hip_check(code):
    if code != 0:
        raise RuntimeError(f"HIP runtime call failed with code {code}")


def _device_array(keep, a, size=None):
    if size is not None and a.size != size:
        raise ValueError(f"array has {a.size} entries, expected {size}")
    p = C.c_void_p()
    _hip_check(_hip().hipMalloc(C.byref(p), C.c_size_t(max(a.nbytes, 8))))
    keep.append(p.value)
    if a.nbytes:
        _hip_check(_hip().hipMemcpy(p, C.c_void_p(a.ctypes.data), C.c_size_t(a.nbytes), 1))
    return p.value


def device_count():
    return int(load_library().nkp_device_count())


def last_error():
    return load_library().nkp_last_error().decode()


def column_coords(ind_i, ind_j, col_start, coupled_tracer_cnt=1):
    first = np.asarray(col_start[:-1], np.int64)
    ci = np.tile(np.asarray(ind_i)[first], coupled_tracer_cnt).astype(np.int32)
    cj = np.tile(np.asarray(ind_j)[first], coupled_tracer_cnt).astype(np.int32)
    return ci, cj


def column_blocks(col_start, tracer_state_len, coupled_tracer_cnt=1):
    col_start = np.asarray(col_start, np.int64)
    parts = [col_start[:-1] + t * tracer_state_len for t in range(coupled_tracer_cnt)]
    return np.concatenate(parts + [np.array([coupled_tracer_cnt * tracer_state_len])]).astype(np.int32)
```

Measured before the change: 33.76 million.

## Overlap Arnoldi host hand-over with next multilevel cycle entry and fuse glue kernels

In each FGMRES Arnoldi step, a new kernel finishes the Hessenberg column, reduces the norm, and writes the column straight to pinned host memory, with an event recorded right after it. The host waits on that event while the GPU goes on: it normalises the next basis vector fused with the level-0 gather, zeroes x, and runs the first smoother half-sweep of the next preconditioner cycle. The goal is to hide the host sync latency and drop a memcpy, a fill and a partials-sum launch per step. The coarse-level restriction is also fused with zeroing the coarse solution. This adds cross-step state (ml.entered) that must be reset on every exit path.

```diff
diff --git a/include/nkp.h b/include/nkp.h
--- a/include/nkp.h
+++ b/include/nkp.h
@@ -86,6 +86,7 @@
    int spmv_diag;
    int ml_lane_fused;
    int dist_smooth_exchange;
+   int step_glue;
 } nkp_tuning;
 
 int nkp_default_tuning (nkp_tuning *t);
diff --git a/nk_ocn_tracer_jacobian_precond_amd/csrc/blas1.hip b/nk_ocn_tracer_jacobian_precond_amd/csrc/blas1.hip
--- a/nk_ocn_tracer_jacobian_precond_amd/csrc/blas1.hip
+++ b/nk_ocn_tracer_jacobian_precond_amd/csrc/blas1.hip
@@ -220,7 +220,7 @@
    const int g = red_grid (n);
    if (v_f32) hipLaunchKernelGGL ((update_w_kernel<float, float2>), dim3 (g), dim3 (B1_THREADS), 0, st, (const float *) V, ld, k, h, w, n, partial, -1.0);
    else hipLaunchKernelGGL ((update_w_kernel<double, double2>), dim3 (g), dim3 (B1_THREADS), 0, st, (const double *) V, ld, k, h, w, n, partial, -1.0);
-   hipLaunchKernelGGL (sum_partials_kernel, dim3 (1), dim3 (NKP_WAVE), 0, st, partial, g, out_nrm2);
+   if (out_nrm2) hipLaunchKernelGGL (sum_partials_kernel, dim3 (1), dim3 (NKP_WAVE), 0, st, partial, g, out_nrm2);
 }
 
 void launch_update_w_group (int R, const GsGroup &G, int64_t ld, int k, const double *msg, int64_t n, double *nrm2, hipStream_t st)
@@ -478,6 +478,31 @@
    hipLaunchKernelGGL (finish_column_pythagoras_kernel, dim3 (1), dim3 (NKP_WAVE), 0, st, h, k, inv);
 }
 
+__global__ __launch_bounds__ (NKP_WAVE)
+void finish_column_host_kernel (double *__restrict__ h, const double *__restrict__ h2, int k, const double *__restrict__ partial, int nblk,
+                                double *__restrict__ nrm2_out, double *__restrict__ inv, double *__restrict__ host_col)
+{
+   double s = 0.0;
+   for (int b = threadIdx.x; b < nblk; b += NKP_WAVE) s += partial[b];
+   s = wave_sum (s);
+   if (h2)
+      for (int j = threadIdx.x; j < k; j += NKP_WAVE) h[j] += h2[j];
+   if (threadIdx.x == 0) {
+      nrm2_out[0] = s;
+      const double t = sqrt (s);
+      h[k] = t;
+      inv[0] = (t > 0.0) ? 1.0 / t : 0.0;
+   }
+   __syncthreads ();
+   for (int j = threadIdx.x; j <= k; j += NKP_WAVE) host_col[j] = h[j];
+   __threadfence_system ();
+}
+
+void launch_finish_column_host (double *h, const double *h2, int k, const double *partial, int64_t n, double *nrm2_out, double *inv, double *host_col, hipStream_t st)
+{
+   hipLaunchKernelGGL (finish_column_host_kernel, dim3 (1), dim3 (NKP_WAVE), 0, st, h, h2, k, partial, red_grid (n), nrm2_out, inv, host_col);
+}
+
 void launch_finish_column (double *h, const double *h2, int k, const double *nrm2, double *inv, hipStream_t st)
 {
    hipLaunchKernelGGL (finish_column_kernel, dim3 (1), dim3 (NKP_WAVE), 0, st, h, h2, k, nrm2, inv);
@@ -495,9 +520,37 @@
    }
 }
 
-void launch_restrict_sum (const int *rptr, const int *ridx, const double *fine, double *coarse, int64_t nc, hipStream_t st)
+__global__ __launch_bounds__ (B1_THREADS)
+void restrict_sum_fill_kernel (const int *__restrict__ rptr, const int *__restrict__ ridx, const double *__restrict__ fine,
+                               double *__restrict__ coarse, double *__restrict__ coarse_x, int64_t nc)
+{
+   const int64_t stride = (int64_t) gridDim.x * B1_THREADS;
+   for (int64_t I = (int64_t) blockIdx.x * B1_THREADS + threadIdx.x; I < nc; I += stride) {
+      const int q1 = rptr[I + 1];
+      double acc = 0.0;
+      for (int q0 = rptr[I]; q0 < q1; q0 += 8) {
+         int id[8];
+         double v[8];
+#pragma unroll
+         for (int t = 0; t < 8; t++) id[t] = (q0 + t < q1) ? ridx[q0 + t] : -1;
+#pragma unroll
+         for (int t = 0; t < 8; t++) v[t] = (id[t] >= 0) ? fine[id[t]] : 0.0;
+#pragma unroll
+         for (int t = 0; t < 8; t++)
+            if (q0 + t < q1) acc += v[t];
+      }
+      coarse[I] = acc;
+      coarse_x[I] = 0.0;
+   }
+}
+
+void launch_restrict_sum (const int *rptr, const int *ridx, const double *fine, double *coarse, int64_t nc, hipStream_t st, double *coarse_x)
 {
    if (nc <= 0) return;
+   if (coarse_x) {
+      hipLaunchKernelGGL (restrict_sum_fill_kernel, dim3 (red_grid (nc) * 2), dim3 (B1_THREADS), 0, st, rptr, ridx, fine, coarse, coarse_x, nc);
+      return;
+   }
    hipLaunchKernelGGL (restrict_sum_kernel, dim3 (red_grid (nc) * 2), dim3 (B1_THREADS), 0, st, rptr, ridx, fine, coarse, nc);
 }
 
@@ -534,6 +587,27 @@
 {
    if (n <= 0) return;
    hipLaunchKernelGGL (gather_kernel, dim3 (red_grid (n) * 2), dim3 (B1_THREADS), 0, st, perm, in, out, n, 1);
+}
+
+__global__ __launch_bounds__ (B1_THREADS)
+void cycle_entry_kernel (const int *__restrict__ perm, const double *__restrict__ w, const double *__restrict__ inv,
+                         double *__restrict__ vnext, double *__restrict__ b0, double *__restrict__ x0, int64_t n)
+{
+   const double a = inv[0];
+   const int64_t stride = (int64_t) gridDim.x * B1_THREADS;
+   for (int64_t i = (int64_t) blockIdx.x * B1_THREADS + threadIdx.x; i < n; i += stride) {
+      const int p = perm[i];
+      const double v = w[p] * a;
+      vnext[p] = v;
+      b0[i] = v;
+      x0[i] = 0.0;
+   }
+}
+
+void launch_cycle_entry (const int *perm, const double *w, const double *inv, double *vnext, double *b0, double *x0, int64_t n, hipStream_t st)
+{
+   if (n <= 0) return;
+   hipLaunchKernelGGL (cycle_entry_kernel, dim3 (red_grid (n) * 2), dim3 (B1_THREADS), 0, st, perm, w, inv, vnext, b0, x0, n);
 }
 
 __global__ __launch_bounds__ (B1_THREADS)
diff --git a/nk_ocn_tracer_jacobian_precond_amd/csrc/inspect.hip b/nk_ocn_tracer_jacobian_precond_amd/csrc/inspect.hip
--- a/nk_ocn_tracer_jacobian_precond_amd/csrc/inspect.hip
+++ b/nk_ocn_tracer_jacobian_precond_amd/csrc/inspect.hip
@@ -153,6 +153,11 @@
       const int prc = valprod_time_prepare (s, arg, which);
       if (prc) return prc;
    }
+   StepEvent step_ev;
+   if (which == 2) {
+      const int erc = step_ev.make (s);
+      if (erc) return erc;
+   }
    hipEvent_t e0, e1;
    HIPCHK (hipEventCreate (&e0));
    HIPCHK (hipEventCreate (&e1));
@@ -176,7 +181,10 @@
          else if (which == 0) spmv_op (s, s->t1, s->t2, nullptr, 0);
          else if (which == 8) launch_diag_spmv (s->A, s->t1, s->t2, nullptr, 0, s->stream);
          else if (which == 1) apply_precond_once (s, s->t1, s->t2);
-         else if (which == 2) arnoldi_step_device (s, arg);
+         else if (which == 2) {
+            const int src = arnoldi_hand_over (s, arg, step_ev.ev);
+            if (src) { s->ml.entered = 0; return src; }
+         }
          else if (which == 5) valgrad_time_launch (s, arg);
          else if (which == 6) valprod_time_launch (s, arg);
          else if (which == 7) valprod_time_composition (s, arg);
@@ -190,6 +198,7 @@
    }
    (void) hipEventDestroy (e0);
    (void) hipEventDestroy (e1);
-   HIPCHK (hipGetLastError ());
-   return NKP_OK;
-}
+   s->ml.entered = 0;
+   HIPCHK (hipGetLastError ());
+   return NKP_OK;
+}
diff --git a/nk_ocn_tracer_jacobian_precond_amd/csrc/krylov.hip b/nk_ocn_tracer_jacobian_precond_amd/csrc/krylov.hip
--- a/nk_ocn_tracer_jacobian_precond_amd/csrc/krylov.hip
+++ b/nk_ocn_tracer_jacobian_precond_amd/csrc/krylov.hip
@@ -73,6 +73,11 @@
    const int64_t ld = s->ld;
    double *zj = s->Z + (int64_t) j * ld;
    const double *vj = s->vf32 ? s->vcur : s->V + (int64_t) j * ld;
+   if (s->ml.entered) {
+      ml_finish (s->ml, zj, s->stream);
+      spmv_op (s, zj, s->w, nullptr, 0);
+      return;
+   }
    if (s->equil) {
       launch_vmul (vj, s->rinv, s->eqtmp, s->n, s->stream);
       apply_precond (s, s->eqtmp, zj);
@@ -84,32 +89,72 @@
    }
 }
 
-void arnoldi_orthogonalise (nkp_solver *s, int j)
+static void arnoldi_column (nkp_solver *s, int j, double *host_col = nullptr)
 {
    const int64_t ld = s->ld;
    launch_multi_dot (s->V, s->vf32, ld, j + 1, s->w, s->n, s->partial, s->h_dev (), s->stream);
    allreduce_dev (s, s->h_dev (), j + 2, 0);
-   launch_update_w (s->V, s->vf32, ld, j + 1, s->h_dev (), s->w, s->n, s->partial, s->misc_dev (), s->stream);
+   launch_update_w (s->V, s->vf32, ld, j + 1, s->h_dev (), s->w, s->n, s->partial, host_col && !s->opt.reorth ? nullptr : s->misc_dev (), s->stream);
    if (s->opt.reorth) {
       launch_multi_dot (s->V, s->vf32, ld, j + 1, s->w, s->n, s->partial, s->h2_dev (), s->stream);
       allreduce_dev (s, s->h2_dev (), j + 2, 0);
-      launch_update_w (s->V, s->vf32, ld, j + 1, s->h2_dev (), s->w, s->n, s->partial, s->misc_dev (), s->stream);
+      launch_update_w (s->V, s->vf32, ld, j + 1, s->h2_dev (), s->w, s->n, s->partial, host_col ? nullptr : s->misc_dev (), s->stream);
       allreduce_dev (s, s->misc_dev (), 1, 0);
-      launch_finish_column (s->h_dev (), s->h2_dev (), j + 1, s->misc_dev (), s->misc_dev () + 1, s->stream);
+      if (host_col) launch_finish_column_host (s->h_dev (), s->h2_dev (), j + 1, s->partial, s->n, s->misc_dev (), s->misc_dev () + 1, host_col, s->stream);
+      else launch_finish_column (s->h_dev (), s->h2_dev (), j + 1, s->misc_dev (), s->misc_dev () + 1, s->stream);
    } else if (s->dist.on && s->tune.dist_one_reduce) {
       launch_finish_column_pythagoras (s->h_dev (), j + 1, s->misc_dev () + 1, s->stream);
-   } else {
+   } else if (host_col) launch_finish_column_host (s->h_dev (), nullptr, j + 1, s->partial, s->n, s->misc_dev (), s->misc_dev () + 1, host_col, s->stream);
+   else {
       allreduce_dev (s, s->misc_dev (), 1, 0);
       launch_finish_column (s->h_dev (), nullptr, j + 1, s->misc_dev (), s->misc_dev () + 1, s->stream);
    }
+}
+
+static void arnoldi_normalise (nkp_solver *s, int j)
+{
+   const int64_t ld = s->ld;
    if (s->vf32) launch_scale_to (s->w, s->misc_dev () + 1, s->vcur, (float *) s->V + (int64_t) (j + 1) * ld, s->n, s->stream);
    else launch_scale_to (s->w, s->misc_dev () + 1, s->V + (int64_t) (j + 1) * ld, nullptr, s->n, s->stream);
 }
 
-void arnoldi_step_device (nkp_solver *s, int j)
-{
+void arnoldi_orthogonalise (nkp_solver *s, int j)
+{
+   arnoldi_column (s, j);
+   arnoldi_normalise (s, j);
+}
+
+static bool step_enters_cycle (const nkp_solver *s)
+{
+   return s->opt.precond == NKP_PRECOND_MULTILEVEL && !s->dist.on && !s->vf32 && !s->equil && s->steps_now == 1 &&
+          !s->ml.lev.empty () && s->ml.lev[0].n == s->n;
+}
+
+int arnoldi_hand_over (nkp_solver *s, int j, hipEvent_t ev)
+{
+   const bool early = ev && (s->tune.step_glue & 8) && j + 1 < s->m && !s->dist.on && !s->equil && s->steps_now == 1;
    arnoldi_apply (s, j);
-   arnoldi_orthogonalise (s, j);
+   arnoldi_column (s, j, early ? s->hpin : nullptr);
+   if (early) HIPCHK (hipEventRecord (ev, s->stream));
+   if (early && step_enters_cycle (s)) ml_enter (s->ml, s->w, s->misc_dev () + 1, s->V + (int64_t) (j + 1) * s->ld, s->stream);
+   else arnoldi_normalise (s, j);
+   if (early) HIPCHK (hipEventSynchronize (ev));
+   else {
+      HIPCHK (hipMemcpyAsync (s->hpin, s->h_dev (), (size_t) (j + 2) * sizeof (double), hipMemcpyDeviceToHost, s->stream));
+      HIPCHK (hipStreamSynchronize (s->stream));
+   }
+   return NKP_OK;
+}
+
+int StepEvent::make (const nkp_solver *s)
+{
+   if (!ev && (s->tune.step_glue & 8) && !s->dist.on) HIPCHK (hipEventCreateWithFlags (&ev, hipEventDisableTiming | hipEventReleaseToSystem));
+   return NKP_OK;
+}
+
+StepEvent::~StepEvent ()
+{
+   if (ev) (void) hipEventDestroy (ev);
 }
 
 
@@ -163,6 +208,7 @@
    hipStream_t st = s->stream;
    const int64_t n = s->n;
    int rc;
+   s->ml.entered = 0;
    spmv_op (s, s->x, s->r, s->b, 1);
    double r2 = 0.0;
    if ((rc = dot_host (s, s->r, s->r, &r2))) return rc;
@@ -224,20 +270,21 @@
 static int fgmres (nkp_solver *s, int *iters_out, double *relres_out)
 {
    FgmresState F;
+   StepEvent ev;
    int rc = fg_begin (s, F);
    if (rc) return rc;
+   if ((rc = ev.make (s))) return rc;
    while (!F.finished) {
       if ((rc = fg_restart (s, F))) return rc;
       if (F.finished) break;
       for (;;) {
-         arnoldi_step_device (s, F.j);
-         HIPCHK (hipMemcpyAsync (s->hpin, s->h_dev (), (size_t) (F.j + 2) * sizeof (double), hipMemcpyDeviceToHost, s->stream));
-         HIPCHK (hipStreamSynchronize (s->stream));
+         if ((rc = arnoldi_hand_over (s, F.j, ev.ev))) { s->ml.entered = 0; return rc; }
          if (s->comm_failed) return fail (NKP_ECOMM, "nkp_solve: a collective of the distributed solve failed (Arnoldi step %d)", F.its + 1);
          if (fg_post_step (s, F)) break;
       }
       if ((rc = fg_end_cycle (s, F))) return rc;
    }
+   s->ml.entered = 0;
    HIPCHK (hipGetLastError ());
    *iters_out = F.its;
    *relres_out = F.relres;
diff --git a/nk_ocn_tracer_jacobian_precond_amd/csrc/mlcycle.hip b/nk_ocn_tracer_jacobian_precond_amd/csrc/mlcycle.hip
--- a/nk_ocn_tracer_jacobian_precond_amd/csrc/mlcycle.hip
+++ b/nk_ocn_tracer_jacobian_precond_amd/csrc/mlcycle.hip
@@ -40,10 +40,31 @@
    for (int step = 0; step < 2; step++) gs_half (H, V, reverse ? 1 - step : step, fused, st);
 }
 
-static void ml_cycle (MlHierarchy &H, int l, hipStream_t st)
+static void first_half_sweep (MlHierarchy &H, MlLevel &V, bool fused, hipStream_t st)
+{
+   if (fused) {
+      if (V.wave_fused) column_solves (H, V, 0, V.b, V.x2, 0, st);
+      else launch_colblock_apply_lanes (V.B, V.color_grp[0], V.color_grp[1], V.b, V.x2, 0, st);
+      V.cur[0] = 1;
+      after_half_sweep (H, V, 0, V.x2, 1, st);
+   } else {
+      column_solves (H, V, 0, V.b, V.x, 0, st);
+      after_half_sweep (H, V, 0, V.x, 1, st);
+   }
+}
+
+static inline bool ml_level_fills_x (const MlHierarchy &H, int l)
+{
+   if (l == H.tail_from) return false;
+   return !(l == (int) H.lev.size () - 1 && H.coarse_inv);
+}
+
+enum { ML_FRESH = 0, ML_FILLED = 1, ML_SOLVED = 2 };
+
+static void ml_cycle (MlHierarchy &H, int l, hipStream_t st, int started = ML_FRESH)
 {
    MlLevel &V = H.lev[l];
-   V.cur[0] = V.cur[1] = 0;
+   if (started != ML_SOLVED) V.cur[0] = V.cur[1] = 0;
    if (l == 0) H.hook_left = 0;
    if (l == H.tail_from && H.coarse_inv && H.gamma_to <= H.gamma_from && ml_tail_launch (H, l, st) == 0) return;
    if (l == (int) H.lev.size () - 1) {
@@ -53,7 +74,7 @@
          return;
       }
       const int sweeps = H.tune->ml_coarsest_sweeps > 0 ? H.tune->ml_coarsest_sweeps : 30;
-      launch_fill (V.x, 0.0, V.n, st);
+      if (started == ML_FRESH) launch_fill (V.x, 0.0, V.n, st);
       column_solves (H, V, 0, V.b, V.x, 0, st);
       gs_half (H, V, 1, false, st);
       for (int s = 1; s < sweeps; s++) gs_sweep (H, V, s & 1, false, st);
@@ -62,26 +83,18 @@
    const bool fused = ml_level_fused (H, V);
    const int nu = (l >= H.coarse_from) ? H.nu_coarse : H.nu;
    if (l == 0 && H.hook) H.hook_left = 4 * nu;
-   launch_fill (V.x, 0.0, V.n, st);
-   if (fused) {
-      if (V.wave_fused) column_solves (H, V, 0, V.b, V.x2, 0, st);
-      else launch_colblock_apply_lanes (V.B, V.color_grp[0], V.color_grp[1], V.b, V.x2, 0, st);
-      V.cur[0] = 1;
-      after_half_sweep (H, V, 0, V.x2, 1, st);
-      gs_half (H, V, 1, true, st);
-   } else {
-      column_solves (H, V, 0, V.b, V.x, 0, st);
-      after_half_sweep (H, V, 0, V.x, 1, st);
-      gs_half (H, V, 1, false, st);
-   }
+   if (started == ML_FRESH) launch_fill (V.x, 0.0, V.n, st);
+   if (started != ML_SOLVED) first_half_sweep (H, V, fused, st);
+   gs_half (H, V, 1, fused, st);
    for (int s = 1; s < nu; s++) gs_sweep (H, V, false, fused, st);
    MlLevel &C = H.lev[l + 1];
    const int gamma = (l >= H.gamma_from && l < H.gamma_to) ? 2 : 1;
    for (int g = 0; g < gamma; g++) {
       if (V.L.dg_val) launch_diag_residual (V.L, V.color_tile[0], V.color_tile[2], V.xnow (), V.b, V.r, st);
       else launch_csr_spmv (V.L, V.xnow (), V.r, V.b, 1, st);
-      launch_restrict_sum (V.rptr, V.ridx, V.r, C.b, V.nc, st);
-      ml_cycle (H, l + 1, st);
+      const bool fill = (H.tune->step_glue & 4) && ml_level_fills_x (H, l + 1);
+      launch_restrict_sum (V.rptr, V.ridx, V.r, C.b, V.nc, st, fill ? C.x : nullptr);
+      ml_cycle (H, l + 1, st, fill ? ML_FILLED : ML_FRESH);
       launch_prolong_add (V.cmap, C.xnow (), V.xnow (), V.n, H.omega, st);
    }
    for (int s = 0; s < nu; s++) gs_sweep (H, V, true, fused, st);
@@ -94,6 +107,28 @@
    H.hook = hook;
    ml_cycle (H, 0, st);
    H.hook = nullptr;
+   launch_scatter (H.perm0, V.xnow (), z, V.n, st);
+}
+
+void ml_enter (MlHierarchy &H, const double *w, const double *inv, double *vnext, hipStream_t st)
+{
+   MlLevel &V = H.lev[0];
+   launch_cycle_entry (H.perm0, w, inv, vnext, V.b, V.x, V.n, st);
+   H.entered = ML_FILLED;
+   if (H.lev.size () >= 2 && H.tail_from != 0) {
+      V.cur[0] = V.cur[1] = 0;
+      H.hook_left = 0;
+      first_half_sweep (H, V, ml_level_fused (H, V), st);
+      H.entered = ML_SOLVED;
+   }
+}
+
+void ml_finish (MlHierarchy &H, double *z, hipStream_t st)
+{
+   MlLevel &V = H.lev[0];
+   const int started = H.entered;
+   H.entered = ML_FRESH;
+   ml_cycle (H, 0, st, started);
    launch_scatter (H.perm0, V.xnow (), z, V.n, st);
 }
 
diff --git a/nk_ocn_tracer_jacobian_precond_amd/csrc/multilevel.h b/nk_ocn_tracer_jacobian_precond_amd/csrc/multilevel.h
--- a/nk_ocn_tracer_jacobian_precond_amd/csrc/multilevel.h
+++ b/nk_ocn_tracer_jacobian_precond_amd/csrc/multilevel.h
@@ -40,6 +40,7 @@
    std::vector<MlLevel> lev;
    const MlSmoothHook *hook = nullptr;
    int hook_left = 0;
+   int entered = 0;
    int *perm0 = nullptr;
    double *coarse_inv = nullptr;
    float *coarse_invf = nullptr;
@@ -77,6 +78,8 @@
 inline int ml_level0_sweeps (const MlHierarchy &H) { return 0 >= H.coarse_from ? H.nu_coarse : H.nu; }
 inline bool ml_level0_hookable (const MlHierarchy &H) { return H.lev.size () >= 2 && H.tail_from != 0 && ml_level0_sweeps (H) > 0; }
 void ml_apply (MlHierarchy &H, const double *r, double *z, hipStream_t st, const MlSmoothHook *hook = nullptr);
+void ml_enter (MlHierarchy &H, const double *w, const double *inv, double *vnext, hipStream_t st);
+void ml_finish (MlHierarchy &H, double *z, hipStream_t st);
 int ml_batch_prepare (MlHierarchy &H, int K);
 void ml_apply_batch (MlHierarchy &H, int K, const double *r, double *z, hipStream_t st);
 void ml_apply_batch_split (MlHierarchy &H, int K, const double *const *src, double *z, double *const *dst, hipStream_t st, const double *src_scale = nullptr);
diff --git a/nk_ocn_tracer_jacobian_precond_amd/csrc/nkp_dev.h b/nk_ocn_tracer_jacobian_precond_amd/csrc/nkp_dev.h
--- a/nk_ocn_tracer_jacobian_precond_amd/csrc/nkp_dev.h
+++ b/nk_ocn_tracer_jacobian_precond_amd/csrc/nkp_dev.h
@@ -246,6 +246,7 @@
 void launch_berr (const double *r, const double *den, int64_t n, double *partial, double *out, hipStream_t st);
 void launch_count_entries (const double *x, int64_t n, double *partial, double *out, hipStream_t st);
 void launch_finish_column (double *h, const double *h2, int k, const double *nrm2, double *inv, hipStream_t st);
+void launch_finish_column_host (double *h, const double *h2, int k, const double *partial, int64_t n, double *nrm2_out, double *inv, double *host_col, hipStream_t st);
 void launch_finish_column_pythagoras (double *h, int k, double *inv, hipStream_t st);
 struct GsGroup {
    const double *V[NKP_BATCH_MAX];
@@ -262,7 +263,8 @@
 void launch_vmul (const double *x, const double *w, double *y, int64_t n, hipStream_t st);
 void launch_fill (double *y, double v, int64_t n, hipStream_t st);
 
-void launch_restrict_sum (const int *rptr, const int *ridx, const double *fine, double *coarse, int64_t nc, hipStream_t st);
+void launch_restrict_sum (const int *rptr, const int *ridx, const double *fine, double *coarse, int64_t nc, hipStream_t st, double *coarse_x = nullptr);
+void launch_cycle_entry (const int *perm, const double *w, const double *inv, double *vnext, double *b0, double *x0, int64_t n, hipStream_t st);
 void launch_prolong_add (const int *cmap, const double *coarse, double *fine, int64_t nf, double omega, hipStream_t st);
 void launch_gather (const int *perm, const double *in, double *out, int64_t n, hipStream_t st);
 void launch_scatter (const int *perm, const double *in, double *out, int64_t n, hipStream_t st);
diff --git a/nk_ocn_tracer_jacobian_precond_amd/csrc/solver_impl.h b/nk_ocn_tracer_jacobian_precond_amd/csrc/solver_impl.h
--- a/nk_ocn_tracer_jacobian_precond_amd/csrc/solver_impl.h
+++ b/nk_ocn_tracer_jacobian_precond_amd/csrc/solver_impl.h
@@ -236,7 +236,12 @@
 NKP_PRIVATE void spmv_op (nkp_solver *s, const double *x, double *y, const double *b, int mode);
 NKP_PRIVATE void arnoldi_apply (nkp_solver *s, int j);
 NKP_PRIVATE void arnoldi_orthogonalise (nkp_solver *s, int j);
-NKP_PRIVATE void arnoldi_step_device (nkp_solver *s, int j);
+NKP_PRIVATE int arnoldi_hand_over (nkp_solver *s, int j, hipEvent_t ev);
+struct NKP_PRIVATE StepEvent {
+   hipEvent_t ev = nullptr;
+   int make (const nkp_solver *s);
+   ~StepEvent ();
+};
 NKP_PRIVATE int fg_begin (nkp_solver *s, FgmresState &F);
 NKP_PRIVATE int fg_restart (nkp_solver *s, FgmresState &F);
 NKP_PRIVATE bool fg_post_step (nkp_solver *s, FgmresState &F);
diff --git a/nk_ocn_tracer_jacobian_precond_amd/csrc/tuning.cpp b/nk_ocn_tracer_jacobian_precond_amd/csrc/tuning.cpp
--- a/nk_ocn_tracer_jacobian_precond_amd/csrc/tuning.cpp
+++ b/nk_ocn_tracer_jacobian_precond_amd/csrc/tuning.cpp
@@ -58,7 +58,7 @@
    t->spmv_variant = 4; t->spmv_compress = 0; t->spmv_pipe_min = 1024; t->spmv_run = 1; t->spmv_wgs = 256;
    t->rhs_batch = 1; t->batch_spmv_rows = 1; t->precond_steps = 0; t->equil = -1; t->dist_overlap = 1; t->dist_ras = 1; t->dist_one_reduce = 0; t->force_dist = 0; t->setup_threads = 0; t->plan_times = 0;
    t->ml_drop_intertracer = 0; t->ml_huge_from = -1; t->dist_ras_rings = 1; t->ml_diag = 32; t->spmv_diag = 32;
-   t->ml_lane_fused = 50000; t->dist_smooth_exchange = 0;
+   t->ml_lane_fused = 50000; t->dist_smooth_exchange = 0; t->step_glue = 12;
 }
 
 const nkp_tuning &nkp_builtin_tuning ()
@@ -104,6 +104,7 @@
    ENV_INT ("NKP_SPMV_DIAG", spmv_diag);
    ENV_INT ("NKP_ML_LANE_FUSED", ml_lane_fused);
    ENV_INT ("NKP_DIST_SMOOTH_EXCHANGE", dist_smooth_exchange);
+   ENV_INT ("NKP_STEP_GLUE", step_glue);
 #undef ENV_INT
 #undef ENV_POS
 #undef ENV_FLAG
diff --git a/nk_ocn_tracer_jacobian_precond_amd/solver.py b/nk_ocn_tracer_jacobian_precond_amd/solver.py
--- a/nk_ocn_tracer_jacobian_precond_amd/solver.py
+++ b/nk_ocn_tracer_jacobian_precond_amd/solver.py
@@ -53,6 +53,7 @@
         ("setup_threads", C.c_int), ("plan_times", C.c_int), ("ml_drop_intertracer", C.c_int), ("dist_one_reduce", C.c_int), ("ml_huge_from", C.c_int), ("col_ldsres_min", C.c_int), ("col_sort_groups", C.c_int), ("batch_spmv_rows", C.c_int),
         ("dist_ras_rings", C.c_int), ("ml_diag", C.c_int), ("spmv_diag", C.c_int), ("ml_lane_fused", C.c_int),
         ("dist_smooth_exchange", C.c_int),
+        ("step_glue", C.c_int),
     ]
 
 
```

Result: faster. 34.42 million, median of 6 (+2.0%).
